# indrajeetadityaroy9/rabitq-ann-search

Hardware: AMD Instinct MI355X
Metric: qps (search_batch_device, layer-0 hot path end to end) + fastscan_dist_per_s (higher is better)
Workload: dtype u32 popcount / f32; 1 GPU; SIFT1M-class synthetic (int-valued, clustered; SURVEY 8d C2): 1000000x128 f32 (D=128), 4-bit RaBitQ FastScan + exact-L2 rerank, R=32, k=10, 10000 queries per GPU resident in HBM; n_index=1000000, dim=128, bits=4, k=10, nq_per_gpu=10000, index_builder=cphnsw_mi355x (this repo), batch_sets=2, parallelism=query-sharded x1, index replicated

## Files before the change

include/cphnsw_mi355x.h:

```cpp
#ifndef CPHNSW_MI355X_H
#define CPHNSW_MI355X_H

#include <stddef.h>
#include <stdint.h>

#ifdef __cplusplus
extern "C" {
#endif

typedef struct cph_index cph_index;

typedef enum {
    CPH_OK = 0,
    CPH_INVALID_ARGUMENT = 1,
    CPH_RUNTIME_ERROR = 2,
    CPH_OUT_OF_MEMORY = 3,
    CPH_NOT_IMPLEMENTED = 4
} cph_status;

const char* cph_last_error(void);

int cph_version(void);

int cph_create(uint64_t dim, uint64_t bits, int device, cph_index** out);
int cph_destroy(cph_index* h);

int cph_load(cph_index* h, const char* path);
int cph_save(cph_index* h, const char* path);
int cph_save_native(cph_index* h, const char* path);
int cph_load_native(cph_index* h, const char* path);
int cph_size(cph_index* h, uint64_t* n);
int cph_dim(cph_index* h, uint64_t* dim);
int cph_is_finalized(cph_index* h, int* flag);

int cph_build(cph_index* h, const float* vectors, uint64_t n);
int cph_finalize(cph_index* h);
int cph_knn_bruteforce(int device, const float* vectors, uint64_t n, uint64_t dim, const float* queries,
                       uint64_t nq, uint32_t* ids, float* dist);

int cph_encode_edges(int device, uint64_t dim, uint64_t bits, const float* parent, const float* nbrs, uint64_t cnt,
                     uint8_t* values, float* aux, uint32_t* pops);

int cph_select_hook(int device, const float* x, uint64_t n, uint64_t D, uint32_t vertex, const uint32_t* fwd,
                    const uint32_t* rev, uint64_t n_rev, uint32_t R, float alpha, float tau, float alpha_max,
                    const float* err, uint32_t* out_ids, uint32_t* out_cnt);

int cph_calib_hook(cph_index* h, const float* queries, const uint32_t* start, uint64_t ns, float* rec, uint32_t* rec_cnt,
                   float* dqp);

int cph_debug_heap_ops(int device, const uint8_t* ops, uint64_t n_ops, const float* keys, const uint32_t* ids, uint64_t n_push,
                       float* out_keys, uint32_t* out_ids, uint32_t* out_size);

int cph_search_batch(cph_index* h, const float* queries, uint64_t n, uint64_t k,
                     int64_t* ids, float* dist);

int cph_search_batch_device(cph_index* h, const float* d_queries, uint64_t n, uint64_t k,
                            int64_t* d_ids, float* d_dist, void* stream);
int cph_synchronize(cph_index* h);

typedef struct cph_filter cph_filter;
int cph_filter_create(cph_index* h, const uint32_t* words, uint64_t n_bits, cph_filter** out);
int cph_filter_destroy(cph_filter* f);
int cph_search_batch_filtered(cph_index* h, const float* queries, uint64_t n, uint64_t k, const cph_filter* f,
                              int64_t* ids, float* dist);
int cph_search_batch_device_filtered(cph_index* h, const float* d_queries, uint64_t n, uint64_t k,
                                     const cph_filter* f, int64_t* d_ids, float* d_dist, void* stream);

int cph_search_batch_exact(cph_index* h, const float* queries, uint64_t n, uint64_t k, const cph_filter* f,
                           int64_t* ids, float* dist);
int cph_search_batch_exact_device(cph_index* h, const float* d_queries, uint64_t n, uint64_t k, const cph_filter* f,
                                  int64_t* d_ids, float* d_dist, void* stream);
int cph_set_exact_threshold(cph_index* h, uint64_t max_allowed);

typedef struct cph_range cph_range;
int cph_range_search_begin(cph_index* h, const void* queries, int queries_on_device, uint64_t n, const float* radius_host,
                           const cph_filter* filter, int exact, uint64_t max_results, void* stream, cph_range** out,
                           uint64_t* total);
int cph_range_search_finish(cph_range* r, int64_t* lims_host, void* ids, void* dist, int results_on_device);
int cph_range_destroy(cph_range* r);
int cph_host_range_plan(uint64_t candidates, uint64_t n_queries, int num_cus, uint64_t* out);
int cph_host_range_tiles(const int64_t* lims, uint64_t n, uint64_t budget_bytes, uint64_t* starts_out, uint64_t* n_tiles_out);
int cph_host_range_merge_pass(const uint64_t* in, uint64_t* out, uint64_t len, uint64_t width);

int cph_search_batch_filters(cph_index* h, const float* queries, uint64_t n, uint64_t k, const cph_filter* const* filters,
                             uint32_t n_filters, const int32_t* filter_of, int exact, int64_t* ids, float* dist);
int cph_search_batch_filters_device(cph_index* h, const float* d_queries, uint64_t n, uint64_t k,
                                    const cph_filter* const* filters, uint32_t n_filters, const int32_t* filter_of, int exact,
                                    int64_t* d_ids, float* d_dist, void* stream);

int cph_filter_create_rows(cph_index* h, const uint32_t* words, uint64_t n_bits, cph_filter** out);

int cph_has_row_map(cph_index* h, int* flag);
int cph_get_row_map(cph_index* h, uint64_t first, uint64_t count, uint32_t* out);
int cph_set_row_map(cph_index* h, const uint32_t* rows, uint64_t n);
enum { CPH_IDS_INTERNAL = 0, CPH_IDS_INPUT = 1 };
int cph_set_result_ids(cph_index* h, int space);

int cph_remove(cph_index* h, const int64_t* ids, uint64_t m, int space, uint64_t* newly);
int cph_live_count(cph_index* h, uint64_t* n);
int cph_get_removed(cph_index* h, uint32_t* words);
int cph_compact(cph_index* h, int64_t* old_to_new);

int cph_search(cph_index* h, const float* query, uint64_t k, int64_t* ids, float* dist,
               uint64_t* m);

int cph_get_vectors(cph_index* h, uint64_t first, uint64_t count, float* out);

int cph_set_batch_sets(cph_index* h, uint32_t n_sets);

int cph_set_search_params(cph_index* h, uint32_t slots, uint64_t beam_capacity);

int cph_last_search_stats(cph_index* h, uint64_t out[12]);
int cph_last_query_expansions(cph_index* index, uint32_t* out, uint64_t n);
int cph_order_queries(cph_index* index, const float* keys, uint64_t n, uint32_t* order);

typedef struct cph_multi cph_multi;
int cph_multi_create(uint64_t dim, uint64_t bits, const int* devices, uint32_t n_dev, cph_multi** out);
int cph_multi_destroy(cph_multi* m);
int cph_multi_load(cph_multi* m, const char* path);
int cph_multi_load_native(cph_multi* m, const char* path);
int cph_multi_save(cph_multi* m, const char* path);
int cph_multi_save_native(cph_multi* m, const char* path);
int cph_multi_build(cph_multi* m, const float* vectors, uint64_t n);
int cph_multi_finalize(cph_multi* m);
int cph_multi_size(cph_multi* m, uint64_t* n);
int cph_multi_is_finalized(cph_multi* m, int* flag);
int cph_multi_search_batch(cph_multi* m, const float* queries, uint64_t n, uint64_t k, int64_t* ids, float* dist);
int cph_multi_search_batch_filtered(cph_multi* m, const float* queries, uint64_t n, uint64_t k,
                                    const cph_filter* const* f, int64_t* ids, float* dist);
int cph_multi_search_batch_exact(cph_multi* m, const float* queries, uint64_t n, uint64_t k,
                                 const cph_filter* const* f, int64_t* ids, float* dist);
int cph_multi_search_batch_filters(cph_multi* m, const float* queries, uint64_t n, uint64_t k, const cph_filter* const* filters,
                                   uint32_t n_filters, const int32_t* filter_of, int exact, int64_t* ids, float* dist);
typedef struct cph_multi_range cph_multi_range;
int cph_multi_range_search_begin(cph_multi* m, const float* queries, uint64_t n, const float* radius_host,
                                 const cph_filter* const* f, int exact, uint64_t max_results, cph_multi_range** out,
                                 uint64_t* total);
int cph_multi_range_search_finish(cph_multi_range* r, int64_t* lims_host, int64_t* ids, float* dist);
int cph_multi_range_destroy(cph_multi_range* r);
int cph_multi_set_exact_threshold(cph_multi* m, uint64_t max_allowed);
int cph_multi_search(cph_multi* m, const float* query, uint64_t k, int64_t* ids, float* dist, uint64_t* count);
int cph_multi_has_row_map(cph_multi* m, int* flag);
int cph_multi_set_row_map(cph_multi* m, const uint32_t* rows, uint64_t n);
int cph_multi_set_result_ids(cph_multi* m, int space);
int cph_multi_set_min_shard(cph_multi* m, uint64_t q);
int cph_multi_last_search_stats(cph_multi* m, uint64_t out[12]);
int cph_multi_last_query_expansions(cph_multi* m, uint32_t* out, uint64_t n);
int cph_multi_remove(cph_multi* m, const int64_t* ids, uint64_t cnt, int space, uint64_t* newly);
int cph_multi_live_count(cph_multi* m, uint64_t* n);
int cph_multi_get_removed(cph_multi* m, uint32_t* words);
int cph_multi_compact(cph_multi* m, int64_t* old_to_new);
int cph_multi_num_replicas(cph_multi* m, uint32_t* n);
int cph_multi_replica(cph_multi* m, uint32_t i, cph_index** out);

typedef struct cph_parts cph_parts;
typedef struct cph_parts_filter cph_parts_filter;
int cph_parts_create(uint64_t dim, uint64_t bits, const int* devices, uint32_t n_dev, cph_parts** out);
int cph_parts_destroy(cph_parts* m);
int cph_parts_build(cph_parts* m, const float* vectors, uint64_t n);
int cph_parts_finalize(cph_parts* m);
int cph_parts_size(cph_parts* m, uint64_t* n);
int cph_parts_is_finalized(cph_parts* m, int* flag);
int cph_parts_save_native(cph_parts* m, const char* path);
int cph_parts_load_native(cph_parts* m, const char* path);
int cph_parts_search_batch(cph_parts* m, const float* queries, uint64_t n, uint64_t k, int64_t* ids, float* dist);
int cph_parts_search_batch_filtered(cph_parts* m, const float* queries, uint64_t n, uint64_t k, const cph_parts_filter* f,
                                    int64_t* ids, float* dist);
int cph_parts_search_batch_exact(cph_parts* m, const float* queries, uint64_t n, uint64_t k, const cph_parts_filter* f,
                                 int64_t* ids, float* dist);
int cph_parts_search_batch_filters(cph_parts* m, const float* queries, uint64_t n, uint64_t k,
                                   const cph_parts_filter* const* filters, uint32_t n_filters, const int32_t* filter_of, int exact,
                                   int64_t* ids, float* dist);
int cph_parts_search_batch_device(cph_parts* m, const float* d_queries, uint64_t n, uint64_t k, int64_t* d_ids, float* d_dist,
                                  void* stream);
int cph_parts_search_batch_device_filtered(cph_parts* m, const float* d_queries, uint64_t n, uint64_t k, const cph_parts_filter* f,
                                           int64_t* d_ids, float* d_dist, void* stream);
int cph_parts_search_batch_exact_device(cph_parts* m, const float* d_queries, uint64_t n, uint64_t k, const cph_parts_filter* f,
                                        int64_t* d_ids, float* d_dist, void* stream);
int cph_parts_search_batch_filters_device(cph_parts* m, const float* d_queries, uint64_t n, uint64_t k,
                                          const cph_parts_filter* const* filters, uint32_t n_filters, const int32_t* filter_of,
                                          int exact, int64_t* d_ids, float* d_dist, void* stream);
int cph_parts_search(cph_parts* m, const float* query, uint64_t k, int64_t* ids, float* dist, uint64_t* count);
int cph_parts_set_exact_threshold(cph_parts* m, uint64_t max_allowed);
int cph_parts_filter_create_rows(cph_parts* m, const uint32_t* words, uint64_t n_bits, cph_parts_filter** out);
int cph_parts_filter_destroy(cph_parts_filter* f);
int cph_parts_last_search_stats(cph_parts* m, uint64_t out[13]);
int cph_parts_last_query_expansions(cph_parts* m, uint32_t* out, uint64_t n);
int cph_parts_remove(cph_parts* m, const int64_t* ids, uint64_t cnt, uint64_t* newly);
int cph_parts_live_count(cph_parts* m, uint64_t* n);
int cph_parts_get_removed(cph_parts* m, uint32_t* words);
int cph_parts_compact(cph_parts* m, int64_t* old_to_new);
int cph_parts_num_parts(cph_parts* m, uint32_t* n);
int cph_parts_part(cph_parts* m, uint32_t i, cph_index** out);
int cph_parts_bounds(cph_parts* m, uint64_t* out);
int cph_merge_rows_hook(int device, const int64_t* ids, const float* dist, uint32_t P, uint64_t n, uint64_t k, const int64_t* lo,
                        int64_t* out_ids, float* out_dist);

int cph_encode_query(cph_index* h, const float* query, uint8_t* lut, float* coeffs);

int cph_entry_point(cph_index* h, const float* query, uint32_t* entry);

int cph_fastscan_block(cph_index* h, const uint8_t* lut, const float* qparams,
                       uint32_t vertex, float dist_qp_sq, float worst, int nn_full,
                       uint32_t* sums, uint32_t* msb, float* est, float* lower,
                       float* lower_stage1);

int cph_exact_l2(cph_index* h, const float* query, const uint32_t* ids, uint64_t n,
                 float* out);

typedef struct cph_stream cph_stream;
int cph_fastscan_stream_create(int device, uint32_t D, uint32_t bits, uint64_t n_blocks,
                               uint64_t seed, cph_stream** out, uint64_t* block_bytes);
int cph_fastscan_stream_run(cph_stream* s, int reps, double* avg_ms, double* checksum);
int cph_fastscan_stream_export(cph_stream* s, uint64_t first, uint64_t count,
                               uint8_t* ref_blocks, uint8_t* lut, float* qparams,
                               float* dist_qp_sq);
int cph_fastscan_stream_eval(cph_stream* s, uint64_t first, uint64_t count, float* est,
                             float* lower);
int cph_fastscan_stream_destroy(cph_stream* s);

int cph_host_rewrite_index(const char* path_in, const char* path_out);
int cph_host_repack_block(uint32_t D, uint32_t bits, const uint8_t* ref_block, uint8_t* dev_block,
                          uint64_t* dev_bytes, uint8_t* ref_roundtrip);
int cph_host_relayout_block(uint32_t D, uint32_t bits, const uint8_t* dev_block, uint8_t* resident_block,
                            uint8_t* dev_roundtrip);
int cph_export_blocks(cph_index* h, uint64_t first, uint64_t count, int resident, uint8_t* out);
int cph_host_encode_query(uint64_t dim, const float* query, uint8_t* lut, float* coeffs, uint32_t* masks);
int cph_host_rows_filter(const uint32_t* words_in, const uint32_t* rows, uint64_t n, uint32_t* words_out);

int cph_host_live_filter(const uint32_t* words_f, const uint32_t* words_removed, uint64_t n, uint32_t* words_out,
                         uint64_t* count_out);

int cph_host_filter_ids(const uint32_t* words, uint64_t n_bits, uint32_t* out_ids, uint64_t* out_count);
int cph_host_exact_plan(uint64_t candidates, uint64_t n_queries, uint64_t k, int num_cus, uint64_t scratch_bytes, uint64_t* out);
int cph_host_filter_groups(const int32_t* filter_of, uint64_t n, const uint64_t* popcounts, uint32_t n_filters, uint64_t k,
                           int exact, uint64_t exact_threshold, uint8_t* routes, uint32_t* perm, uint32_t* seg);
int cph_host_exact_group_plan(const uint64_t* seg_candidates, const uint64_t* seg_queries, uint32_t n_segments, uint64_t k,
                              int num_cus, uint64_t scratch_bytes, uint32_t* items, uint64_t cap_items, uint64_t* out);
int cph_host_part_bounds(uint64_t n, uint32_t P, uint64_t* out);

#ifdef __cplusplus
}
#endif
#endif
```

rabitq-ann-search_amd/cphnsw_mi355x/_lib.py:

```python
import ctypes as C
import importlib.util
import os
import sys

from . import build as _build

OK, INVALID_ARGUMENT, RUNTIME_ERROR, OUT_OF_MEMORY, NOT_IMPLEMENTED = range(5)
IDS_INTERNAL, IDS_INPUT = 0, 1

SYMBOLS = {
    "cph_last_error": (C.c_char_p, []),
    "cph_version": (C.c_int, []),
    "cph_create": (C.c_int, [C.c_uint64, C.c_uint64, C.c_int, C.POINTER(C.c_void_p)]),
    "cph_destroy": (C.c_int, [C.c_void_p]),
    "cph_load": (C.c_int, [C.c_void_p, C.c_char_p]),
    "cph_save": (C.c_int, [C.c_void_p, C.c_char_p]),
    "cph_save_native": (C.c_int, [C.c_void_p, C.c_char_p]),
    "cph_load_native": (C.c_int, [C.c_void_p, C.c_char_p]),
    "cph_size": (C.c_int, [C.c_void_p, C.POINTER(C.c_uint64)]),
    "cph_dim": (C.c_int, [C.c_void_p, C.POINTER(C.c_uint64)]),
    "cph_is_finalized": (C.c_int, [C.c_void_p, C.POINTER(C.c_int)]),
    "cph_build": (C.c_int, [C.c_void_p, C.c_void_p, C.c_uint64]),
    "cph_finalize": (C.c_int, [C.c_void_p]),
    "cph_knn_bruteforce": (C.c_int, [C.c_int, C.c_void_p, C.c_uint64, C.c_uint64, C.c_void_p, C.c_uint64,
                                     C.c_void_p, C.c_void_p]),
    "cph_debug_heap_ops": (C.c_int, [C.c_int, C.c_void_p, C.c_uint64, C.c_void_p, C.c_void_p, C.c_uint64, C.c_void_p, C.c_void_p,
                                     C.c_void_p]),
    "cph_select_hook": (C.c_int, [C.c_int, C.c_void_p, C.c_uint64, C.c_uint64, C.c_uint32, C.c_void_p, C.c_void_p, C.c_uint64,
                                  C.c_uint32, C.c_float, C.c_float, C.c_float, C.c_void_p, C.c_void_p, C.c_void_p]),
    "cph_calib_hook": (C.c_int, [C.c_void_p, C.c_void_p, C.c_void_p, C.c_uint64, C.c_void_p, C.c_void_p, C.c_void_p]),
    "cph_encode_edges": (C.c_int, [C.c_int, C.c_uint64, C.c_uint64, C.c_void_p, C.c_void_p, C.c_uint64, C.c_void_p,
                                   C.c_void_p, C.c_void_p]),
    "cph_search_batch": (C.c_int, [C.c_void_p, C.c_void_p, C.c_uint64, C.c_uint64, C.c_void_p, C.c_void_p]),
    "cph_search_batch_device": (C.c_int, [C.c_void_p, C.c_void_p, C.c_uint64, C.c_uint64, C.c_void_p,
                                          C.c_void_p, C.c_void_p]),
    "cph_filter_create": (C.c_int, [C.c_void_p, C.c_void_p, C.c_uint64, C.POINTER(C.c_void_p)]),
    "cph_filter_destroy": (C.c_int, [C.c_void_p]),
    "cph_search_batch_filtered": (C.c_int, [C.c_void_p, C.c_void_p, C.c_uint64, C.c_uint64, C.c_void_p, C.c_void_p,
                                            C.c_void_p]),
    "cph_search_batch_device_filtered": (C.c_int, [C.c_void_p, C.c_void_p, C.c_uint64, C.c_uint64, C.c_void_p,
                                                   C.c_void_p, C.c_void_p, C.c_void_p]),
    "cph_search_batch_exact": (C.c_int, [C.c_void_p, C.c_void_p, C.c_uint64, C.c_uint64, C.c_void_p, C.c_void_p,
                                         C.c_void_p]),
    "cph_search_batch_exact_device": (C.c_int, [C.c_void_p, C.c_void_p, C.c_uint64, C.c_uint64, C.c_void_p,
                                                C.c_void_p, C.c_void_p, C.c_void_p]),
    "cph_set_exact_threshold": (C.c_int, [C.c_void_p, C.c_uint64]),
    "cph_search_batch_filters": (C.c_int, [C.c_void_p, C.c_void_p, C.c_uint64, C.c_uint64, C.c_void_p, C.c_uint32,
                                           C.c_void_p, C.c_int, C.c_void_p, C.c_void_p]),
    "cph_search_batch_filters_device": (C.c_int, [C.c_void_p, C.c_void_p, C.c_uint64, C.c_uint64, C.c_void_p, C.c_uint32,
                                                  C.c_void_p, C.c_int, C.c_void_p, C.c_void_p, C.c_void_p]),
    "cph_multi_search_batch_filters": (C.c_int, [C.c_void_p, C.c_void_p, C.c_uint64, C.c_uint64, C.c_void_p, C.c_uint32,
                                                 C.c_void_p, C.c_int, C.c_void_p, C.c_void_p]),
    "cph_host_filter_groups": (C.c_int, [C.c_void_p, C.c_uint64, C.c_void_p, C.c_uint32, C.c_uint64, C.c_int, C.c_uint64,
                                         C.c_void_p, C.c_void_p, C.c_void_p]),
    "cph_host_exact_group_plan": (C.c_int, [C.c_void_p, C.c_void_p, C.c_uint32, C.c_uint64, C.c_int, C.c_uint64, C.c_void_p,
                                            C.c_uint64, C.c_void_p]),
    "cph_multi_search_batch_exact": (C.c_int, [C.c_void_p, C.c_void_p, C.c_uint64, C.c_uint64, C.c_void_p,
                                               C.c_void_p, C.c_void_p]),
    "cph_multi_set_exact_threshold": (C.c_int, [C.c_void_p, C.c_uint64]),
    "cph_host_filter_ids": (C.c_int, [C.c_void_p, C.c_uint64, C.c_void_p, C.POINTER(C.c_uint64)]),
    "cph_host_exact_plan": (C.c_int, [C.c_uint64, C.c_uint64, C.c_uint64, C.c_int, C.c_uint64, C.POINTER(C.c_uint64)]),
    "cph_range_search_begin": (C.c_int, [C.c_void_p, C.c_void_p, C.c_int, C.c_uint64, C.c_void_p, C.c_void_p, C.c_int, C.c_uint64,
                                         C.c_void_p, C.POINTER(C.c_void_p), C.POINTER(C.c_uint64)]),
    "cph_range_search_finish": (C.c_int, [C.c_void_p, C.c_void_p, C.c_void_p, C.c_void_p, C.c_int]),
    "cph_range_destroy": (C.c_int, [C.c_void_p]),
    "cph_multi_range_search_begin": (C.c_int, [C.c_void_p, C.c_void_p, C.c_uint64, C.c_void_p, C.c_void_p, C.c_int, C.c_uint64,
                                               C.POINTER(C.c_void_p), C.POINTER(C.c_uint64)]),
    "cph_multi_range_search_finish": (C.c_int, [C.c_void_p, C.c_void_p, C.c_void_p, C.c_void_p]),
    "cph_multi_range_destroy": (C.c_int, [C.c_void_p]),
    "cph_host_range_plan": (C.c_int, [C.c_uint64, C.c_uint64, C.c_int, C.POINTER(C.c_uint64)]),
    "cph_host_range_tiles": (C.c_int, [C.c_void_p, C.c_uint64, C.c_uint64, C.c_void_p, C.POINTER(C.c_uint64)]),
    "cph_host_range_merge_pass": (C.c_int, [C.c_void_p, C.c_void_p, C.c_uint64, C.c_uint64]),
    "cph_filter_create_rows": (C.c_int, [C.c_void_p, C.c_void_p, C.c_uint64, C.POINTER(C.c_void_p)]),
    "cph_has_row_map": (C.c_int, [C.c_void_p, C.POINTER(C.c_int)]),
    "cph_get_row_map": (C.c_int, [C.c_void_p, C.c_uint64, C.c_uint64, C.c_void_p]),
    "cph_set_row_map": (C.c_int, [C.c_void_p, C.c_void_p, C.c_uint64]),
    "cph_set_result_ids": (C.c_int, [C.c_void_p, C.c_int]),
    "cph_remove": (C.c_int, [C.c_void_p, C.c_void_p, C.c_uint64, C.c_int, C.POINTER(C.c_uint64)]),
    "cph_live_count": (C.c_int, [C.c_void_p, C.POINTER(C.c_uint64)]),
    "cph_get_removed": (C.c_int, [C.c_void_p, C.c_void_p]),
    "cph_compact": (C.c_int, [C.c_void_p, C.c_void_p]),
    "cph_host_live_filter": (C.c_int, [C.c_void_p, C.c_void_p, C.c_uint64, C.c_void_p, C.POINTER(C.c_uint64)]),
    "cph_multi_remove": (C.c_int, [C.c_void_p, C.c_void_p, C.c_uint64, C.c_int, C.POINTER(C.c_uint64)]),
    "cph_multi_live_count": (C.c_int, [C.c_void_p, C.POINTER(C.c_uint64)]),
    "cph_multi_get_removed": (C.c_int, [C.c_void_p, C.c_void_p]),
    "cph_multi_compact": (C.c_int, [C.c_void_p, C.c_void_p]),
    "cph_parts_remove": (C.c_int, [C.c_void_p, C.c_void_p, C.c_uint64, C.POINTER(C.c_uint64)]),
    "cph_parts_live_count": (C.c_int, [C.c_void_p, C.POINTER(C.c_uint64)]),
    "cph_parts_get_removed": (C.c_int, [C.c_void_p, C.c_void_p]),
    "cph_parts_compact": (C.c_int, [C.c_void_p, C.c_void_p]),
    "cph_synchronize": (C.c_int, [C.c_void_p]),
    "cph_set_batch_sets": (C.c_int, [C.c_void_p, C.c_uint32]),
    "cph_search": (C.c_int, [C.c_void_p, C.c_void_p, C.c_uint64, C.c_void_p, C.c_void_p,
                             C.POINTER(C.c_uint64)]),
    "cph_get_vectors": (C.c_int, [C.c_void_p, C.c_uint64, C.c_uint64, C.c_void_p]),
    "cph_set_search_params": (C.c_int, [C.c_void_p, C.c_uint32, C.c_uint64]),
    "cph_last_search_stats": (C.c_int, [C.c_void_p, C.POINTER(C.c_uint64)]),
    "cph_last_query_expansions": (C.c_int, [C.c_void_p, C.c_void_p, C.c_uint64]),
    "cph_order_queries": (C.c_int, [C.c_void_p, C.c_void_p, C.c_uint64, C.c_void_p]),
    "cph_multi_create": (C.c_int, [C.c_uint64, C.c_uint64, C.c_void_p, C.c_uint32, C.POINTER(C.c_void_p)]),
    "cph_multi_destroy": (C.c_int, [C.c_void_p]),
    "cph_multi_load": (C.c_int, [C.c_void_p, C.c_char_p]),
    "cph_multi_load_native": (C.c_int, [C.c_void_p, C.c_char_p]),
    "cph_multi_save": (C.c_int, [C.c_void_p, C.c_char_p]),
    "cph_multi_save_native": (C.c_int, [C.c_void_p, C.c_char_p]),
    "cph_multi_build": (C.c_int, [C.c_void_p, C.c_void_p, C.c_uint64]),
    "cph_multi_finalize": (C.c_int, [C.c_void_p]),
    "cph_multi_size": (C.c_int, [C.c_void_p, C.POINTER(C.c_uint64)]),
    "cph_multi_is_finalized": (C.c_int, [C.c_void_p, C.POINTER(C.c_int)]),
    "cph_multi_search_batch": (C.c_int, [C.c_void_p, C.c_void_p, C.c_uint64, C.c_uint64, C.c_void_p, C.c_void_p]),
    "cph_multi_search_batch_filtered": (C.c_int, [C.c_void_p, C.c_void_p, C.c_uint64, C.c_uint64, C.c_void_p,
                                                  C.c_void_p, C.c_void_p]),
    "cph_multi_search": (C.c_int, [C.c_void_p, C.c_void_p, C.c_uint64, C.c_void_p, C.c_void_p,
                                   C.POINTER(C.c_uint64)]),
    "cph_multi_has_row_map": (C.c_int, [C.c_void_p, C.POINTER(C.c_int)]),
    "cph_multi_set_row_map": (C.c_int, [C.c_void_p, C.c_void_p, C.c_uint64]),
    "cph_multi_set_result_ids": (C.c_int, [C.c_void_p, C.c_int]),
    "cph_multi_set_min_shard": (C.c_int, [C.c_void_p, C.c_uint64]),
    "cph_multi_last_search_stats": (C.c_int, [C.c_void_p, C.POINTER(C.c_uint64)]),
    "cph_multi_last_query_expansions": (C.c_int, [C.c_void_p, C.c_void_p, C.c_uint64]),
    "cph_multi_num_replicas": (C.c_int, [C.c_void_p, C.POINTER(C.c_uint32)]),
    "cph_multi_replica": (C.c_int, [C.c_void_p, C.c_uint32, C.POINTER(C.c_void_p)]),
    "cph_parts_create": (C.c_int, [C.c_uint64, C.c_uint64, C.c_void_p, C.c_uint32, C.POINTER(C.c_void_p)]),
    "cph_parts_destroy": (C.c_int, [C.c_void_p]),
    "cph_parts_build": (C.c_int, [C.c_void_p, C.c_void_p, C.c_uint64]),
    "cph_parts_finalize": (C.c_int, [C.c_void_p]),
    "cph_parts_size": (C.c_int, [C.c_void_p, C.POINTER(C.c_uint64)]),
    "cph_parts_is_finalized": (C.c_int, [C.c_void_p, C.POINTER(C.c_int)]),
    "cph_parts_save_native": (C.c_int, [C.c_void_p, C.c_char_p]),
    "cph_parts_load_native": (C.c_int, [C.c_void_p, C.c_char_p]),
    "cph_parts_search_batch": (C.c_int, [C.c_void_p, C.c_void_p, C.c_uint64, C.c_uint64, C.c_void_p, C.c_void_p]),
    "cph_parts_search_batch_filtered": (C.c_int, [C.c_void_p, C.c_void_p, C.c_uint64, C.c_uint64, C.c_void_p, C.c_void_p,
                                                  C.c_void_p]),
    "cph_parts_search_batch_exact": (C.c_int, [C.c_void_p, C.c_void_p, C.c_uint64, C.c_uint64, C.c_void_p, C.c_void_p,
                                               C.c_void_p]),
    "cph_parts_search_batch_filters": (C.c_int, [C.c_void_p, C.c_void_p, C.c_uint64, C.c_uint64, C.c_void_p, C.c_uint32,
                                                 C.c_void_p, C.c_int, C.c_void_p, C.c_void_p]),
    "cph_parts_search_batch_device": (C.c_int, [C.c_void_p, C.c_void_p, C.c_uint64, C.c_uint64, C.c_void_p, C.c_void_p,
                                                C.c_void_p]),
    "cph_parts_search_batch_device_filtered": (C.c_int, [C.c_void_p, C.c_void_p, C.c_uint64, C.c_uint64, C.c_void_p,
                                                         C.c_void_p, C.c_void_p, C.c_void_p]),
    "cph_parts_search_batch_exact_device": (C.c_int, [C.c_void_p, C.c_void_p, C.c_uint64, C.c_uint64, C.c_void_p,
                                                      C.c_void_p, C.c_void_p, C.c_void_p]),
    "cph_parts_search_batch_filters_device": (C.c_int, [C.c_void_p, C.c_void_p, C.c_uint64, C.c_uint64, C.c_void_p, C.c_uint32,
                                                        C.c_void_p, C.c_int, C.c_void_p, C.c_void_p, C.c_void_p]),
    "cph_parts_search": (C.c_int, [C.c_void_p, C.c_void_p, C.c_uint64, C.c_void_p, C.c_void_p, C.POINTER(C.c_uint64)]),
    "cph_parts_set_exact_threshold": (C.c_int, [C.c_void_p, C.c_uint64]),
    "cph_parts_filter_create_rows": (C.c_int, [C.c_void_p, C.c_void_p, C.c_uint64, C.POINTER(C.c_void_p)]),
    "cph_parts_filter_destroy": (C.c_int, [C.c_void_p]),
    "cph_parts_last_search_stats": (C.c_int, [C.c_void_p, C.POINTER(C.c_uint64)]),
    "cph_parts_last_query_expansions": (C.c_int, [C.c_void_p, C.c_void_p, C.c_uint64]),
    "cph_parts_num_parts": (C.c_int, [C.c_void_p, C.POINTER(C.c_uint32)]),
    "cph_parts_part": (C.c_int, [C.c_void_p, C.c_uint32, C.POINTER(C.c_void_p)]),
    "cph_parts_bounds": (C.c_int, [C.c_void_p, C.c_void_p]),
    "cph_merge_rows_hook": (C.c_int, [C.c_int, C.c_void_p, C.c_void_p, C.c_uint32, C.c_uint64, C.c_uint64, C.c_void_p,
                                      C.c_void_p, C.c_void_p]),
    "cph_host_part_bounds": (C.c_int, [C.c_uint64, C.c_uint32, C.c_void_p]),
    "cph_encode_query": (C.c_int, [C.c_void_p, C.c_void_p, C.c_void_p, C.c_void_p]),
    "cph_entry_point": (C.c_int, [C.c_void_p, C.c_void_p, C.POINTER(C.c_uint32)]),
    "cph_fastscan_block": (C.c_int, [C.c_void_p, C.c_void_p, C.c_void_p, C.c_uint32, C.c_float, C.c_float,
                                     C.c_int, C.c_void_p, C.c_void_p, C.c_void_p, C.c_void_p, C.c_void_p]),
    "cph_exact_l2": (C.c_int, [C.c_void_p, C.c_void_p, C.c_void_p, C.c_uint64, C.c_void_p]),
    "cph_host_rewrite_index": (C.c_int, [C.c_char_p, C.c_char_p]),
    "cph_host_repack_block": (C.c_int, [C.c_uint32, C.c_uint32, C.c_void_p, C.c_void_p, C.POINTER(C.c_uint64), C.c_void_p]),
    "cph_host_relayout_block": (C.c_int, [C.c_uint32, C.c_uint32, C.c_void_p, C.c_void_p, C.c_void_p]),
    "cph_export_blocks": (C.c_int, [C.c_void_p, C.c_uint64, C.c_uint64, C.c_int, C.c_void_p]),
    "cph_host_encode_query": (C.c_int, [C.c_uint64, C.c_void_p, C.c_void_p, C.c_void_p, C.c_void_p]),
    "cph_host_rows_filter": (C.c_int, [C.c_void_p, C.c_void_p, C.c_uint64, C.c_void_p]),
    "cph_fastscan_stream_create": (C.c_int, [C.c_int, C.c_uint32, C.c_uint32, C.c_uint64, C.c_uint64,
                                             C.POINTER(C.c_void_p), C.POINTER(C.c_uint64)]),
    "cph_fastscan_stream_run": (C.c_int, [C.c_void_p, C.c_int, C.POINTER(C.c_double), C.POINTER(C.c_double)]),
    "cph_fastscan_stream_export": (C.c_int, [C.c_void_p, C.c_uint64, C.c_uint64, C.c_void_p, C.c_void_p,
                                             C.c_void_p, C.POINTER(C.c_float)]),
    "cph_fastscan_stream_eval": (C.c_int, [C.c_void_p, C.c_uint64, C.c_uint64, C.c_void_p, C.c_void_p]),
    "cph_fastscan_stream_destroy": (C.c_int, [C.c_void_p]),
}

_LIB = None


def _share_hip_runtime_with_torch():
    if "torch" in sys.modules:
        return
    try:
        spec = importlib.util.find_spec("torch")
    except (ImportError, ValueError):
        spec = None
    if spec is None or not spec.origin:
        return
    cand = os.path.join(os.path.dirname(spec.origin), "lib", "libamdhip64.so")
    if os.path.exists(cand):
        try:
            C.CDLL(cand, mode=C.RTLD_GLOBAL)
        except OSError:
            pass


def lib():
    global _LIB
    if _LIB is None:
        path = os.environ.get("CPH_LIB_PATH")
        if not path:
            path = _build.LIB_PATH
            if _build.needs_build():
                path = _build.build_library()
        _share_hip_runtime_with_torch()
        L = C.CDLL(path)
        diagnostic = bool(os.environ.get("CPH_LIB_PATH"))
        for name, (res, args) in SYMBOLS.items():
            try:
                fn = getattr(L, name)
            except AttributeError:
                if diagnostic:
                    continue
                raise
            fn.restype = res
            fn.argtypes = args
        _LIB = L
    return _LIB


def check(rc):
    if rc == OK:
        return
    msg = lib().cph_last_error().decode("utf-8", "replace")
    if rc == INVALID_ARGUMENT:
        raise ValueError(msg)
    if rc == OUT_OF_MEMORY:
        raise MemoryError(msg)
    if rc == NOT_IMPLEMENTED:
        raise NotImplementedError(msg)
    raise RuntimeError(msg)
```

rabitq-ann-search_amd/cphnsw_mi355x/index.py:

```python
import ctypes as C

import numpy as np

from . import _lib

DEFAULT_K = 10


def _as_f32(a):
    return np.ascontiguousarray(np.asarray(a), dtype=np.float32)


def pack_allowed_bits(mask):
    m = np.asarray(mask, dtype=bool).ravel()
    nw = (m.size + 31) // 32
    padded = np.zeros(nw * 32, dtype=np.uint64)
    padded[:m.size] = m
    return (padded.reshape(nw, 32) << np.arange(32, dtype=np.uint64)).sum(axis=1).astype(np.uint32)


class IdFilter:

    def __init__(self, index, words, n_bits, count, input_rows=False):
        self._h = C.c_void_p()
# ... 610 lines not shown
        st = np.ascontiguousarray(start, np.uint32)
        ns = q.shape[0]
        rec = np.zeros((ns, 32, 6), np.float32)
        cnt = np.zeros(ns, np.uint32)
        dqp = np.zeros(ns, np.float32)
        _lib.check(_lib.lib().cph_calib_hook(self._h, q.ctypes.data, st.ctypes.data, ns, rec.ctypes.data, cnt.ctypes.data,
                                             dqp.ctypes.data))
        return rec, cnt, dqp

    def save_native(self, path):
        if self._p is not None:
            _lib.check(_lib.lib().cph_parts_save_native(self._p, str(path).encode()))
            return
        if self._m is not None:
            _lib.check(_lib.lib().cph_multi_save_native(self._m, str(path).encode()))
            return
        _lib.check(_lib.lib().cph_save_native(self._h, str(path).encode()))

    def load_native(self, path):
        if self._p is not None:
            _lib.check(_lib.lib().cph_parts_load_native(self._p, str(path).encode()))
            return
        try:
            if self._m is not None:
                _lib.check(_lib.lib().cph_multi_load_native(self._m, str(path).encode()))
                return
            _lib.check(_lib.lib().cph_load_native(self._h, str(path).encode()))
        finally:
            self._after_index_change()

    def _after_index_change(self):
        if self._result_ids == "input" and not self.has_row_map:
            self.result_ids = "internal"

    @property
    def has_row_map(self):
        f = C.c_int(0)
        if self._p is not None:
            return self.is_finalized
        if self._m is not None:
            _lib.check(_lib.lib().cph_multi_has_row_map(self._m, C.byref(f)))
        else:
            _lib.check(_lib.lib().cph_has_row_map(self._h, C.byref(f)))
        return bool(f.value)

    def row_map(self):
        self._no_parts("row_map")
        out = np.empty(self.size, np.uint32)
        _lib.check(_lib.lib().cph_get_row_map(self._h, 0, out.size, out.ctypes.data))
        return out.astype(np.int64)

    def set_row_map(self, rows):
        self._no_parts("set_row_map")
        if rows is None:
            if self._m is not None:
                _lib.check(_lib.lib().cph_multi_set_row_map(self._m, None, 0))
            else:
                _lib.check(_lib.lib().cph_set_row_map(self._h, None, 0))
            self._result_ids = "internal"
            return
        r = np.asarray(rows)
        if r.ndim != 1 or not np.issubdtype(r.dtype, np.integer):
            raise ValueError("row map must be a 1D integer array")
        if r.size and (r.min() < 0 or r.max() > 0xFFFFFFFF):
            raise ValueError("row map must be a permutation of 0..size-1")
        r = np.ascontiguousarray(r, np.uint32)
        if self._m is not None:
            _lib.check(_lib.lib().cph_multi_set_row_map(self._m, r.ctypes.data, r.size))
        else:
            _lib.check(_lib.lib().cph_set_row_map(self._h, r.ctypes.data, r.size))

    @property
    def result_ids(self):
        return self._result_ids

    @result_ids.setter
    def result_ids(self, space):
        if space not in ("internal", "input"):
            raise ValueError('result_ids must be "internal" or "input"')
        if self._p is not None:
            if space != "input":
                raise ValueError('a partitioned index speaks input rows only: result_ids stays "input" '
                                 "(every part has its own internal ids: part(i))")
            return
        code = _lib.IDS_INPUT if space == "input" else _lib.IDS_INTERNAL
        if self._m is not None:
            _lib.check(_lib.lib().cph_multi_set_result_ids(self._m, code))
        else:
            _lib.check(_lib.lib().cph_set_result_ids(self._h, code))
        self._result_ids = space

    @property
    def exact_threshold(self):
        return self._exact_threshold

    @exact_threshold.setter
    def exact_threshold(self, max_allowed):
        v = int(max_allowed)
        if v < 0:
            raise ValueError("exact_threshold must be >= 0")
        if self._p is not None:
            _lib.check(_lib.lib().cph_parts_set_exact_threshold(self._p, v))
        elif self._m is not None:
            _lib.check(_lib.lib().cph_multi_set_exact_threshold(self._m, v))
        else:
            _lib.check(_lib.lib().cph_set_exact_threshold(self._h, v))
        self._exact_threshold = v

    @property
    def size(self):
        n = C.c_uint64(0)
        if self._p is not None:
            _lib.check(_lib.lib().cph_parts_size(self._p, C.byref(n)))
        elif self._m is not None:
            _lib.check(_lib.lib().cph_multi_size(self._m, C.byref(n)))
        else:
            _lib.check(_lib.lib().cph_size(self._h, C.byref(n)))
        return n.value

    @property
    def dim(self):
        return self._dim

    @property
    def is_finalized(self):
        f = C.c_int(0)
        if self._p is not None:
            _lib.check(_lib.lib().cph_parts_is_finalized(self._p, C.byref(f)))
        elif self._m is not None:
            _lib.check(_lib.lib().cph_multi_is_finalized(self._m, C.byref(f)))
        else:
            _lib.check(_lib.lib().cph_is_finalized(self._h, C.byref(f)))
        return bool(f.value)

    def set_batch_sets(self, n_sets):
        for h in self._replicas():
            _lib.check(_lib.lib().cph_set_batch_sets(h, int(n_sets)))

    def set_search_params(self, slots=0, beam_capacity=0):
        for h in self._replicas():
            _lib.check(_lib.lib().cph_set_search_params(h, int(slots), int(beam_capacity)))

    def last_search_stats(self):
        out = (C.c_uint64 * 13)()
        if self._p is not None:
            _lib.check(_lib.lib().cph_parts_last_search_stats(self._p, out))
        elif self._m is not None:
            _lib.check(_lib.lib().cph_multi_last_search_stats(self._m, out))
        else:
            _lib.check(_lib.lib().cph_last_search_stats(self._h, out))
        keys = ("expansions", "exact_l2", "new_neighbours", "beam_pushes", "stage2_skipped",
                "rerun_queries", "kernel_us", "expansions_nothing_new", "slots", "capacity",
                "stage2_reruns", "stage2_undecided") + (("merge_us",) if self._p is not None else ())
        return dict(zip(keys, [int(x) for x in out]))

    def synchronize(self):
        for h in self._replicas():
            _lib.check(_lib.lib().cph_synchronize(h))

    def last_query_expansions(self, n):
        out = np.empty(int(n), np.uint32)
        if self._p is not None:
            _lib.check(_lib.lib().cph_parts_last_query_expansions(self._p, out.ctypes.data, int(n)))
        elif self._m is not None:
            _lib.check(_lib.lib().cph_multi_last_query_expansions(self._m, out.ctypes.data, int(n)))
        else:
            _lib.check(_lib.lib().cph_last_query_expansions(self._h, out.ctypes.data, int(n)))
        return out

    def order_queries(self, keys):
        self._no_parts("order_queries")
        keys = np.ascontiguousarray(keys, np.float32)
        out = np.empty(len(keys), np.uint32)
        _lib.check(_lib.lib().cph_order_queries(self._h, keys.ctypes.data, len(keys), out.ctypes.data))
        return out

    def get_vectors(self, first=0, count=None):
        self._no_parts("get_vectors")
        if count is None:
            count = self.size - first
        out = np.empty((count, self._dim), np.float32)
        _lib.check(_lib.lib().cph_get_vectors(self._h, int(first), int(count), out.ctypes.data))
        return out

    def internal_to_input_rows(self, base, chunk=1 << 18):
        base = _as_f32(base)
        key = {}
        for i in range(base.shape[0] - 1, -1, -1):
            key[base[i].tobytes()] = i
        out = np.empty(self.size, np.int64)
        for lo in range(0, self.size, chunk):
            v = self.get_vectors(lo, min(chunk, self.size - lo))
            for j in range(v.shape[0]):
                out[lo + j] = key[v[j].tobytes()]
        return out

    def encode_query(self, query):
        self._no_parts("encode_query")
        q = _as_f32(query)
        D = 1
        while D < self._dim:
            D *= 2
        lut = np.zeros((D // 4, 16), np.uint8)
        co = np.zeros(3, np.float32)
        _lib.check(_lib.lib().cph_encode_query(self._h, q.ctypes.data, lut.ctypes.data, co.ctypes.data))
        return lut, co

    def entry_point(self, query):
        self._no_parts("entry_point")
        q = _as_f32(query)
        ep = C.c_uint32(0)
        _lib.check(_lib.lib().cph_entry_point(self._h, q.ctypes.data, C.byref(ep)))
        return ep.value

    def fastscan_block(self, lut, qparams, vertex, dist_qp_sq, worst=3.402823466e+38, nn_full=False):
        self._no_parts("fastscan_block")
        lut = np.ascontiguousarray(lut, np.uint8)
        qp = np.ascontiguousarray(qparams, np.float32)
        sums = np.zeros(32, np.uint32)
        msb = np.zeros(32, np.uint32)
        est = np.zeros(32, np.float32)
        lower = np.zeros(32, np.float32)
        lower1 = np.zeros(32, np.float32)
        _lib.check(_lib.lib().cph_fastscan_block(
            self._h, lut.ctypes.data, qp.ctypes.data, int(vertex), float(dist_qp_sq), float(worst),
            int(bool(nn_full)), sums.ctypes.data, msb.ctypes.data, est.ctypes.data, lower.ctypes.data,
            lower1.ctypes.data))
        return sums, msb, est, lower, lower1

    def exact_l2(self, query, ids):
        self._no_parts("exact_l2")
        q = _as_f32(query)
        ids = np.ascontiguousarray(ids, np.uint32)
        out = np.zeros(len(ids), np.float32)
        _lib.check(_lib.lib().cph_exact_l2(self._h, q.ctypes.data, ids.ctypes.data, len(ids),
                                           out.ctypes.data))
        return out


def knn_bruteforce(vectors, queries=None, device=None):
    v = _as_f32(vectors)
    n, dim = v.shape
    q = None if queries is None else _as_f32(queries)
    if q is not None and (q.ndim != 2 or q.shape[1] != dim):
        raise ValueError("queries must be a (nq, dim) array")
    rows = n if q is None else q.shape[0]
    ids = np.zeros((rows, 32), np.uint32)
    dist = np.zeros((rows, 32), np.float32)
    dev = _default_device() if device is None else int(device)
    _lib.check(_lib.lib().cph_knn_bruteforce(dev, v.ctypes.data, n, dim, None if q is None else q.ctypes.data,
                                             0 if q is None else q.shape[0], ids.ctypes.data, dist.ctypes.data))
    return ids, dist


def encode_edges(parent, nbrs, bits, device=None):
    p = _as_f32(parent)
    nb = _as_f32(nbrs)
    cnt, dim = nb.shape
    D = 16
    while D < dim:
        D *= 2
    vals = np.zeros((cnt, D), np.uint8)
    aux = np.zeros((cnt, 3), np.float32)
    pops = np.zeros((cnt, 2), np.uint32)
    dev = _default_device() if device is None else int(device)
    _lib.check(_lib.lib().cph_encode_edges(dev, dim, int(bits), p.ctypes.data, nb.ctypes.data, cnt, vals.ctypes.data,
                                           aux.ctypes.data, pops.ctypes.data))
    return vals, aux, pops


def select_neighbors_debug(x, vertex, fwd, rev, R, alpha, tau, alpha_max=0.0, err=None, device=None):
    x = _as_f32(x)
    n, D = x.shape
    fwd = np.ascontiguousarray(fwd, np.uint32)
    rev = np.ascontiguousarray(rev, np.uint32)
    assert fwd.shape == (32,)
    out = np.zeros(32, np.uint32)
    cnt = np.zeros(1, np.uint32)
    e = None if err is None else _as_f32(err)
    dev = _default_device() if device is None else int(device)
    _lib.check(_lib.lib().cph_select_hook(dev, x.ctypes.data, n, D, int(vertex), fwd.ctypes.data, rev.ctypes.data if len(rev) else None,
                                          len(rev), int(R), float(alpha), float(tau), float(alpha_max),
                                          None if e is None else e.ctypes.data, out.ctypes.data, cnt.ctypes.data))
    return out[:cnt[0]].copy()


def heap_ops_debug(ops, keys, ids, device=None):
    ops = np.ascontiguousarray(ops, np.uint8)
    keys = np.ascontiguousarray(keys, np.float32)
    ids = np.ascontiguousarray(ids, np.uint32)
    n_push = int((ops != 0).sum())
    assert len(keys) == n_push and len(ids) == n_push
    ok = np.zeros(max(1, n_push), np.float32)
    oi = np.zeros(max(1, n_push), np.uint32)
    sz = np.zeros(1, np.uint32)
    dev = _default_device() if device is None else int(device)
    _lib.check(_lib.lib().cph_debug_heap_ops(dev, ops.ctypes.data, len(ops), keys.ctypes.data, ids.ctypes.data, n_push,
                                             ok.ctypes.data, oi.ctypes.data, sz.ctypes.data))
    return ok[:sz[0]].copy(), oi[:sz[0]].copy()


def _default_device():
    import os
    try:
        return int(os.environ.get("LOCAL_RANK", "0"))
    except ValueError:
        return 0
# ... 46 lines not shown
```

rabitq-ann-search_amd/csrc/cphnsw_mi355x.hip:

```cpp
#include <hip/hip_runtime.h>

#include <algorithm>
#include <atomic>
#include <cfloat>
#include <chrono>
#include <condition_variable>
#include <deque>
#include <functional>
#include <memory>
#include <mutex>
#include <new>
#include <shared_mutex>
#include <string>
#include <thread>
#include <vector>

#include "../../include/cphnsw_mi355x.h"
#include "cph_core.h"
#include "device_buf.h"
#include "device_encode.h"
#include "device_fastscan.h"
#include "device_search.h"
#include "device_stream.h"
#include "device_heap_test.h"
#include "device_relayout.h"
#include "device_rows.h"
#include "device_tombstone.h"
#include "device_exact.h"
#include "device_range.h"
#include "host_index.h"
#include "host_parallel.h"
#include "search_coalescer.h"
#include "multi_device.h"
#include "partitioned.h"
#include "device_merge.h"
#include "native_file.h"
#include "builder_pipeline.h"

using namespace cph;

namespace {

thread_local std::string g_err;

int fail(int code, const std::string& msg) {
    g_err = msg;
    return code;
}

struct InvalidArg : std::invalid_argument {
    using std::invalid_argument::invalid_argument;
};

template <class F>
int guarded(F&& f) {
    try {
        f();
        return CPH_OK;
    } catch (const std::invalid_argument& e) {
        return fail(CPH_INVALID_ARGUMENT, e.what());
    } catch (const std::bad_alloc&) {
        return fail(CPH_OUT_OF_MEMORY, "out of memory");
    } catch (const std::exception& e) {
        return fail(CPH_RUNTIME_ERROR, e.what());
    }
}

size_t next_pow2(size_t n) {
    size_t p = 1;
    while (p < n) p *= 2;
    return p;
}

#define CPH_LAUNCH_BITS(KERNEL, bits, SDV, grid, block, lds, st, args)                            \
    do {                                                                                          \
        if ((bits) == 1) hipLaunchKernelGGL((KERNEL<1, SDV>), grid, block, lds, st, args);        \
        else if ((bits) == 2) hipLaunchKernelGGL((KERNEL<2, SDV>), grid, block, lds, st, args);   \
        else hipLaunchKernelGGL((KERNEL<4, SDV>), grid, block, lds, st, args);                    \
    } while (0)
#define CPH_LAUNCH(KERNEL, bits, D, grid, block, lds, st, args)                                   \
    do {                                                                                          \
        if ((D) == 128) CPH_LAUNCH_BITS(KERNEL, bits, 128, grid, block, lds, st, args);           \
        else if ((D) == 1024) CPH_LAUNCH_BITS(KERNEL, bits, 1024, grid, block, lds, st, args);    \
        else CPH_LAUNCH_BITS(KERNEL, bits, 0, grid, block, lds, st, args);                        \
        HIP_CHECK(hipGetLastError());                                                             \
    } while (0)

__global__ void scan_counts_kernel(const uint8_t* blocks, uint64_t n, uint32_t stride, uint32_t count_off, uint32_t* flags) {
    const uint64_t v = (uint64_t)blockIdx.x * blockDim.x + threadIdx.x;
    if (v >= n) return;
    const uint32_t cnt = *reinterpret_cast<const uint32_t*>(blocks + v * stride + count_off);
    if (cnt & 7u) atomicOr(flags, 2u);
}

}

struct BatchSet {
    DevBuf<float> d_queries_raw, d_queries, d_entry_dist, d_dist;
    DevBuf<uint4> d_qmasks;
    DevBuf<QueryHeader> d_qhdr;
    DevBuf<int64_t> d_ids;
    DevBuf<uint32_t> d_count, d_status, d_order, d_redo;
    DevBuf<unsigned long long> d_stats;
    unsigned long long* pin_stats = nullptr;
    uint8_t* pin_io = nullptr;
    uint8_t* pin_io_dev = nullptr;
    size_t pin_io_bytes = 0;
    DevBuf<uint32_t> d_bitmaps, d_logids;
    DevBuf<uint32_t> d_beam, d_beam_tail;
    uint32_t slots = 0;
    uint64_t cap = 0;
    DevBuf<uint32_t> r_bitmaps, r_logids;
    DevBuf<uint32_t> r_beam, r_beam_tail;
    uint32_t r_slots = 0;
    hipEvent_t ev0 = nullptr, ev1 = nullptr, ev_done = nullptr;
    bool used = false;
    uint32_t nq = 0;
    uint32_t run_slots = 0;
    uint64_t run_cap = 0;
    DevBuf<float> x_qpad, x_qnorm;
    DevBuf<unsigned long long> x_pools;
    DevBuf<uint32_t> x_counts;
    bool stats_in_hbm = false;
    uint8_t* pin_tab = nullptr;
    size_t pin_tab_bytes = 0;
    DevBuf<uint8_t> d_tab;
    DevBuf<uint32_t> d_redo2;
    hipEvent_t ev_tab = nullptr;
    bool tab_used = false;
};
constexpr int kMaxBatchSets = 4;

struct RangeScratch {
    DevBuf<float> d_q, qpad, qnorm, d_rad, g_dist, o_dist;
    DevBuf<int64_t> g_ids, o_ids;
    DevBuf<uint32_t> counts;
    DevBuf<unsigned long long> offs, sums, d_lims, d_stats, arena, arena2;
    DevBuf<uint8_t> d_tab;
};
constexpr size_t kRangeScratchKept = 2;
constexpr uint64_t kSmallBatch = 32;

struct cph_filter {
    int device = 0;
    uint64_t n_bits = 0;
    uint64_t popcount = 0;
    DevBuf<uint32_t> words;
    mutable std::mutex ids_mu;
    mutable DevBuf<uint32_t> ids, ids_scratch;
    mutable hipEvent_t ids_ev = nullptr;
    mutable std::mutex eff_mu;
    mutable std::vector<std::pair<uint64_t, std::shared_ptr<cph_filter>>> eff;
    ~cph_filter() { if (ids_ev) (void)hipEventDestroy(ids_ev); }
};
constexpr size_t kEffCached = 4;
struct EffDeleter {
    void operator()(cph_filter* f) const {
        if (hipSetDevice(f->device) == hipSuccess) (void)hipDeviceSynchronize();
        delete f;
    }
};
static std::atomic<uint64_t> g_removed_epoch{0};

struct cph_index {
    uint64_t dim = 0;
    uint32_t bits = 0;
    uint32_t D = 0;
    int device = 0;
    bool finalized = false;
    bool needs_build = false;
    bool borrowed = false;
    bool host_less = false;
    std::vector<float> pending;
    uint64_t pending_n = 0;
    HostIndex host;
    DevLayout L{};
    SearchConsts sc{};
    uint32_t flags = 0;
    int num_cus = 256;
    bool waves_from_env = false;
    uint32_t waves_per_cu = 4 * CPH_SEARCH_WAVES_PER_SIMD;
    DevBuf<uint8_t> d_blocks;
    DevBuf<float> d_raw, d_norm;
    DevBuf<uint32_t> d_rows;
    bool has_rows = false;
    bool ids_input = false;
    size_t exact_scratch_bytes = (size_t)1 << 30;
    uint64_t exact_threshold = 0;
    DevBuf<uint32_t> d_removed;
    DevBuf<unsigned long long> d_rm_count;
    uint64_t rm_epoch = 0;
    std::shared_ptr<cph_filter> live;
    std::atomic<bool> tombstones{false};
    DevBuf<float> d_signs;
    DevBuf<uint32_t> d_upper;
    DevBuf<uint32_t> d_row_of;
    UpperLayerDev layers[kMaxUpperLayers];
    int32_t dev_max_level = 0;
    float norm_factor = 0.0f, inv_sqrt_d = 0.0f;
    NativeMapping native_map;
    const uint8_t* own_view = nullptr;
    std::vector<uint8_t> own_store;
    BatchSet sets[kMaxBatchSets + kLeaderSlots];
    int n_sets = 2;
    int last_set = kMaxBatchSets - 1;
    int last_search = -1;
    bool last_range = false;
    uint64_t range_exact = 0;
    std::vector<std::unique_ptr<RangeScratch>> range_scratch;
    uint64_t index_epoch = 0;
    hipStream_t own_stream = nullptr;
    bool order_queries = true;
    uint32_t want_slots = 0;
    uint64_t want_cap = 0;
    uint64_t auto_cap = 0;
    bool pf_off = false;
    bool pf_dense = false;
    std::mutex mu;
    SearchCoalescer coal;
    struct LeaderSlot {
        hipStream_t stream = nullptr;
        uint8_t* pin = nullptr;
        uint8_t* pin_dev = nullptr;
        size_t pin_bytes = 0;
        uint32_t seq = 0;
        uint64_t cur_n = 0, cur_k = 0;
    } leaders[kLeaderSlots];

    void use_device() const { HIP_CHECK(hipSetDevice(device)); }
};

namespace {

bool probe_first(const cph_index* h) {
    return (h->L.D == 128 || h->L.D == 1024) && !(h->flags & 2u) && !h->pf_off && !h->pf_dense;
}

uint64_t stage2_stat(const BatchSet& s, StatWord w) {
#if defined(CPH_PHASE_TIMERS) || defined(CPH_TRAFFIC_STATS)
    (void)s; (void)w;
    return 0;
#else
    return s.pin_stats[w];
#endif
}

void reset_adaptation(cph_index* h) {
    h->auto_cap = 0;
    h->pf_off = false;
    h->pf_dense = false;
    h->last_search = -1;
    h->last_range = false;
}

void drop_host_state(cph_index* h) {
    h->needs_build = false;
    std::vector<float>().swap(h->pending);
    h->pending_n = 0;
    h->native_map.reset();
    h->own_view = nullptr;
    std::vector<uint8_t>().swap(h->own_store);
}

void sync_row_map(cph_index* h) {
    const std::vector<uint32_t>& rows = h->host.rows;
    h->has_rows = !rows.empty();
    if (h->has_rows) {
        h->d_rows.alloc(rows.size());
        HIP_CHECK(hipMemcpy(h->d_rows.p, rows.data(), rows.size() * 4, hipMemcpyHostToDevice));
    } else {
        h->d_rows.release();
        h->ids_input = false;
    }
}

hipStream_t own_stream(cph_index* h);

std::shared_ptr<cph_filter> make_live_filter(cph_index* h, const uint32_t* d_allow) {
    const uint64_t n = h->host.n, nw = (n + 31) / 32;
    std::shared_ptr<cph_filter> e(new cph_filter(), EffDeleter());
    e->device = h->device;
    e->n_bits = n;
    e->words.alloc(std::max<uint64_t>(nw, 1));
    h->d_rm_count.alloc(1);
    hipStream_t st = own_stream(h);
    live_filter(d_allow, h->d_removed.p, n, e->words.p, h->d_rm_count.p, st);
    unsigned long long c = 0;
    HIP_CHECK(hipMemcpyAsync(&c, h->d_rm_count.p, 8, hipMemcpyDeviceToHost, st));
    HIP_CHECK(hipStreamSynchronize(st));
    e->popcount = c;
    return e;
}

void sync_removed(cph_index* h) {
    HostIndex& hi = h->host;
    h->rm_epoch = ++g_removed_epoch;
    h->live.reset();
    if (hi.n_removed == 0) {
        std::vector<uint32_t>().swap(hi.removed);
        h->d_removed.release();
        h->tombstones.store(false);
        return;
    }
    h->tombstones.store(true);
    const uint64_t nw = (hi.n + 31) / 32;
    h->d_removed.alloc(nw);
    HIP_CHECK(hipMemcpy(h->d_removed.p, hi.removed.data(), nw * 4, hipMemcpyHostToDevice));
    h->live = make_live_filter(h, nullptr);
}

std::shared_ptr<const cph_filter> effective_filter(cph_index* h, const cph_filter* f) {
    if (h->host.n_removed == 0) return std::shared_ptr<const cph_filter>(std::shared_ptr<const cph_filter>(), f);
    if (!f) {
        if (!h->live) h->live = make_live_filter(h, nullptr);
        return h->live;
    }
    std::lock_guard<std::mutex> lk(f->eff_mu);
    for (auto& e : f->eff)
        if (e.first == h->rm_epoch) return e.second;
    if (f->eff.size() >= kEffCached) f->eff.erase(f->eff.begin());
    std::shared_ptr<cph_filter> e = make_live_filter(h, f->words.p);
    f->eff.emplace_back(h->rm_epoch, e);
    return e;
}

void require_finalized(cph_index* h) {
    if (!h->finalized) throw std::runtime_error("Search failed: invalid entry point after finalize.");
}

void release_scratch(BatchSet& s) {
    s.d_bitmaps.release(); s.d_logids.release(); s.d_beam.release(); s.d_beam_tail.release();
    s.r_bitmaps.release(); s.r_logids.release(); s.r_beam.release(); s.r_beam_tail.release();
    s.x_qpad.release(); s.x_qnorm.release(); s.x_pools.release(); s.x_counts.release();
    s.slots = 0; s.cap = 0; s.r_slots = 0;
}

void quiesce(cph_index* h) {
    for (auto& s : h->sets)
        if (s.used && s.ev_done) HIP_CHECK(hipEventSynchronize(s.ev_done));
}

void upload_arrays(cph_index* h) {
    h->use_device();
    quiesce(h);
    const HostIndex& hi = h->host;
    h->L = make_dev_layout((uint32_t)hi.D, (uint32_t)hi.bw);
    const size_t n = hi.n;
    const size_t stride = h->L.stride;
    h->d_blocks.alloc(n * stride + 64);
    h->d_raw.alloc(n * hi.D);
    h->d_norm.alloc(n);
    const size_t chunk = std::max<size_t>(1, std::min<size_t>(n, (256u << 20) / stride));
    std::vector<uint8_t> stage(chunk * stride);
    for (size_t base = 0; base < n; base += chunk) {
        const size_t cnt = std::min(chunk, n - base);
        parallel_for(cnt, 256, [&](size_t lo, size_t hi_) {
            for (size_t v = lo; v < hi_; ++v)
                repack_ref_to_dev(hi.nb(base + v), hi.RL, h->L, &stage[v * stride]);
        });
        HIP_CHECK(hipMemcpy(h->d_blocks.p + base * stride, stage.data(), cnt * stride,
                            hipMemcpyHostToDevice));
    }
    relayout_blocks(h->d_blocks.p, n, h->L, true);
    HIP_CHECK(hipMemcpy(h->d_raw.p, hi.raw.data(), n * hi.D * 4, hipMemcpyHostToDevice));
    HIP_CHECK(hipMemcpy(h->d_norm.p, hi.norm_sq.data(), n * 4, hipMemcpyHostToDevice));
}

void upload_feeders(cph_index* h) {
    h->use_device();
    quiesce(h);
    const HostIndex& hi = h->host;
    const size_t n = hi.n;
    h->L = make_dev_layout((uint32_t)hi.D, (uint32_t)hi.bw);
    h->sc = hi.consts();
    h->flags = hi.has_dup_neighbors ? 1u : 0u;
    if (n != 0) {
        DevBuf<uint32_t> d_flag(1);
        HIP_CHECK(hipMemset(d_flag.p, 0, 4));
        hipLaunchKernelGGL(scan_counts_kernel, dim3((uint32_t)((n + 255) / 256)), dim3(256), 0, nullptr, h->d_blocks.p, (uint64_t)n,
                           h->L.stride, h->L.count_off, d_flag.p);
        HIP_CHECK(hipGetLastError());
        uint32_t f = 0;
        HIP_CHECK(hipMemcpy(&f, d_flag.p, 4, hipMemcpyDeviceToHost));
        h->flags |= f & 2u;
    }
    h->d_signs.alloc(3 * hi.D);
    HIP_CHECK(hipMemcpy(h->d_signs.p, hi.rot.signs.data(), 3 * hi.D * 4, hipMemcpyHostToDevice));
    const float d = static_cast<float>(hi.D);
    h->norm_factor = 1.0f / (d * std::sqrt(d));
    h->inv_sqrt_d = 1.0f / std::sqrt(d);
    const int nl = std::min<int>({(int)hi.upper.size(), (int)hi.max_level, kMaxUpperLayers});
    h->dev_max_level = hi.max_level > 0 ? nl : 0;
    std::vector<uint32_t> flat;
    std::vector<size_t> off_nodes(nl), off_offs(nl), off_nbrs(nl);
    for (int l = 0; l < nl; ++l) {
        const auto& layer = hi.upper[l];
        off_nodes[l] = flat.size();
        for (const auto& e : layer) flat.push_back(e.node);
        off_offs[l] = flat.size();
        uint32_t acc = 0;
        for (const auto& e : layer) { flat.push_back(acc); acc += (uint32_t)e.nbrs.size(); }
        flat.push_back(acc);
        off_nbrs[l] = flat.size();
        for (const auto& e : layer) flat.insert(flat.end(), e.nbrs.begin(), e.nbrs.end());
    }
    h->d_upper.alloc(flat.size() + 1);
    if (!flat.empty())
        HIP_CHECK(hipMemcpy(h->d_upper.p, flat.data(), flat.size() * 4, hipMemcpyHostToDevice));
    for (int l = 0; l < kMaxUpperLayers; ++l) h->layers[l] = UpperLayerDev{nullptr, nullptr, nullptr, nullptr, 0};
    int mapped = 0;
    for (int l = 0; l < nl; ++l) mapped += hi.upper[l].size() > 16 ? 1 : 0;
    h->d_row_of.alloc((size_t)mapped * n + 1);
    std::vector<uint32_t> row_of;
    for (int l = 0, m = 0; l < nl; ++l) {
        const uint32_t* dmap = nullptr;
        if (hi.upper[l].size() > 16) {
            row_of.assign(n, kInvalidNode);
            uint64_t first = 0;
            bool fits = true;
            for (size_t r = 0; r < hi.upper[l].size(); ++r) {
                const uint64_t deg = hi.upper[l][r].nbrs.size();
                if (first >= (1u << 26) || deg > 62) { fits = false; break; }
                row_of[hi.upper[l][r].node] = (uint32_t)first | ((uint32_t)deg << 26);
                first += deg;
            }
            if (!fits) { h->layers[l] = UpperLayerDev{h->d_upper.p + off_nodes[l], h->d_upper.p + off_offs[l], h->d_upper.p + off_nbrs[l], nullptr, (uint32_t)hi.upper[l].size()}; ++m; continue; }
            HIP_CHECK(hipMemcpy(h->d_row_of.p + (size_t)m * n, row_of.data(), n * 4, hipMemcpyHostToDevice));
            dmap = h->d_row_of.p + (size_t)m * n;
            ++m;
        }
        h->layers[l] = UpperLayerDev{h->d_upper.p + off_nodes[l], h->d_upper.p + off_offs[l],
                                     h->d_upper.p + off_nbrs[l], dmap, (uint32_t)hi.upper[l].size()};
    }
    for (auto& s : h->sets) release_scratch(s);
    reset_adaptation(h);
}

void materialize_search_data(cph_index* h) {
    HostIndex& hi = h->host;
    if (!hi.search_data.empty() || hi.n == 0) return;
    h->use_device();
    quiesce(h);
    const size_t n = hi.n, stride = h->L.stride, own_stride = hi.RL.nb_off;
    hi.search_data.assign(n * hi.RL.vertex_bytes, 0);
    const size_t chunk = std::max<size_t>(1, std::min<size_t>(n, (512u << 20) / stride));
    std::vector<uint8_t> stage(chunk * stride);
    for (size_t base = 0; base < n; base += chunk) {
        const size_t c = std::min(chunk, n - base);
        download_blocks(h->d_blocks.p + base * stride, c, h->L, stage.data());
        parallel_for(c, 256, [&](size_t lo, size_t hi_) {
            for (size_t v = lo; v < hi_; ++v) {
                uint8_t* dst = &hi.search_data[(base + v) * hi.RL.vertex_bytes];
                if (h->own_view) std::memcpy(dst, h->own_view + (base + v) * own_stride, own_stride);
                repack_dev_to_ref(&stage[v * stride], h->L, hi.RL, dst + hi.RL.nb_off);
            }
        });
    }
}

void init_set(BatchSet& s) {
    if (s.ev0) return;
    HIP_CHECK(hipEventCreate(&s.ev0));
    HIP_CHECK(hipEventCreate(&s.ev1));
    HIP_CHECK(hipEventCreateWithFlags(&s.ev_done, hipEventDisableTiming));
    HIP_CHECK(hipHostMalloc(reinterpret_cast<void**>(&s.pin_stats), kStatWords * 8, hipHostMallocDefault));
    std::memset(s.pin_stats, 0, kStatWords * 8);
}

BatchSet& next_set(cph_index* h, hipStream_t st) {
    h->last_set = (h->last_set + 1) % h->n_sets;
    BatchSet& s = h->sets[h->last_set];
    init_set(s);
    for (BatchSet& o : h->sets) {
        if (!(o.used && o.ev_done && !o.stats_in_hbm && hipEventQuery(o.ev_done) == hipSuccess)) continue;
        const uint64_t reruns = o.pin_stats[kStatReruns], stage2_reruns = stage2_stat(o, kStatStage2Reruns);
        if (reruns > stage2_reruns && o.cap < h->host.n + 1)
            h->auto_cap = std::max<uint64_t>(h->auto_cap, std::min<uint64_t>(h->host.n + 1, o.cap * 4));
        if (stage2_reruns * 50 > o.nq) h->pf_off = true;
        if (o.pin_stats[kStatExpansions] >= 10000) {
            const double new_per_exp = (double)o.pin_stats[kStatNew] / (double)o.pin_stats[kStatExpansions];
            const double off = h->bits == 4 ? 6.0 : 2.8, on = h->bits == 4 ? 4.5 : 2.2;
            if (new_per_exp > off) h->pf_dense = true;
            else if (new_per_exp < on) h->pf_dense = false;
        }
    }
    if (s.used) HIP_CHECK(hipStreamWaitEvent(st, s.ev_done, 0));
    return s;
}

void stage_queries(cph_index* h, BatchSet& s, const float* d_raw_q, uint64_t nq, hipStream_t st) {
    const HostIndex& hi = h->host;
    const uint32_t D = (uint32_t)hi.D, PW = h->L.PW;
    if (hi.entry == kInvalidNode || hi.entry >= hi.n)
        throw std::runtime_error("Search failed: invalid entry point after finalize.");
    if (s.d_queries.n < nq * D || s.d_qmasks.n < nq * PW || s.d_qhdr.n < nq) {
        if (s.used) HIP_CHECK(hipEventSynchronize(s.ev_done));
        s.d_queries.alloc(nq * D);
        s.d_qmasks.alloc(nq * PW);
        s.d_qhdr.alloc(nq);
        s.d_entry_dist.alloc(nq);
        s.d_order.alloc(nq);
    }
    EncodeArgs a{};
    a.queries_raw = d_raw_q;
    a.nq = (uint32_t)nq;
    a.dim = (uint32_t)hi.dim;
    a.D = D;
    a.PW = PW;
    a.signs = h->d_signs.p;
    a.norm_factor = h->norm_factor;
    a.inv_sqrt_d = h->inv_sqrt_d;
    a.raw = h->d_raw.p;
    a.n = hi.n;
    a.entry = hi.entry;
    a.max_level = h->dev_max_level;
    for (int l = 0; l < kMaxUpperLayers; ++l) a.layers[l] = h->layers[l];
    a.queries_padded = s.d_queries.p;
    a.qmasks = s.d_qmasks.p;
    a.qhdr = s.d_qhdr.p;
    a.entry_dist = s.d_entry_dist.p;
    const uint32_t grid = (uint32_t)std::min<uint64_t>(nq, (uint64_t)h->num_cus * 32);
    hipLaunchKernelGGL(encode_kernel, dim3(grid), dim3(64), encode_lds_bytes(D), st, a);
    HIP_CHECK(hipGetLastError());
}

const float* upload_queries(cph_index* h, BatchSet& s, const float* queries, uint64_t nq, hipStream_t st) {
    if (s.d_queries_raw.n < nq * h->dim) {
        if (s.used) HIP_CHECK(hipEventSynchronize(s.ev_done));
        s.d_queries_raw.alloc(nq * h->dim);
    }
    HIP_CHECK(hipMemcpyAsync(s.d_queries_raw.p, queries, nq * h->dim * 4, hipMemcpyHostToDevice, st));
    return s.d_queries_raw.p;
}

void ensure_scratch(cph_index* h, BatchSet& s, uint32_t slots, uint64_t cap, hipStream_t st) {
    const uint64_t n = h->host.n;
    const uint64_t bm_words = (n + 31) / 32;
    if (!(s.slots >= slots && s.cap == cap)) {
        if (s.used) HIP_CHECK(hipEventSynchronize(s.ev_done));
        s.d_bitmaps.alloc((size_t)slots * bm_words);
        HIP_CHECK(hipMemsetAsync(s.d_bitmaps.p, 0, (size_t)slots * bm_words * 4, st));
        s.d_logids.alloc((size_t)slots * cap);
        s.d_beam.alloc((size_t)slots * kBeamPagesDwords);
        s.d_beam_tail.alloc((size_t)slots * beam_tail_dwords(cap));
        s.slots = slots;
        s.cap = cap;
    }
    if ((cap < n + 1 || probe_first(h)) && s.r_slots == 0) {
        size_t free_b = 0, total_b = 0;
        HIP_CHECK(hipMemGetInfo(&free_b, &total_b));
        const uint64_t per = (n + 1) * 4 + ((uint64_t)kBeamPagesDwords + beam_tail_dwords(n + 1)) * 4 + bm_words * 4;
        const uint64_t want = (&s - h->sets) >= kMaxBatchSets ? kLeaderGroup : kSmallBatch;
        const uint32_t rs = (uint32_t)std::max<uint64_t>(1, std::min<uint64_t>(want, (uint64_t)(free_b * 0.25) / per));
        s.r_bitmaps.alloc((size_t)rs * bm_words);
        HIP_CHECK(hipMemsetAsync(s.r_bitmaps.p, 0, (size_t)rs * bm_words * 4, st));
        s.r_logids.alloc((size_t)rs * (n + 1));
        s.r_beam.alloc((size_t)rs * kBeamPagesDwords);
        s.r_beam_tail.alloc((size_t)rs * beam_tail_dwords(n + 1));
        s.r_slots = rs;
    }
}

struct DoneFlags {
    uint32_t* flags = nullptr;
    uint32_t seq = 0;
};

enum class Launch {
    Main,
    Rerun,
    Direct,
};

void launch_search_kernel(uint32_t bits, uint32_t D, bool pf, bool filtered, bool table_of_filters, uint32_t grid, size_t lds,
                          hipStream_t st, const SearchArgs& a) {
    using Kernel = void (*)(SearchArgs);
    static const Kernel table[3][3][4] = {
        {{search_kernel<1, 0, true, false>, search_kernel<1, 0, true, false>, search_kernel<1, 0, false, true>,
          search_kernel<1, 0, false, true, true>},
         {search_kernel<1, 128, false, false>, search_kernel<1, 128, true, false>, search_kernel<1, 128, false, true>,
          search_kernel<1, 128, false, true, true>},
         {search_kernel<1, 1024, false, false>, search_kernel<1, 1024, true, false>, search_kernel<1, 1024, false, true>,
          search_kernel<1, 1024, false, true, true>}},
        {{search_kernel<2, 0, true, false>, search_kernel<2, 0, true, false>, search_kernel<2, 0, false, true>,
          search_kernel<2, 0, false, true, true>},
         {search_kernel<2, 128, false, false>, search_kernel<2, 128, true, false>, search_kernel<2, 128, false, true>,
          search_kernel<2, 128, false, true, true>},
         {search_kernel<2, 1024, false, false>, search_kernel<2, 1024, true, false>, search_kernel<2, 1024, false, true>,
          search_kernel<2, 1024, false, true, true>}},
        {{search_kernel<4, 0, true, false>, search_kernel<4, 0, true, false>, search_kernel<4, 0, false, true>,
          search_kernel<4, 0, false, true, true>},
         {search_kernel<4, 128, false, false>, search_kernel<4, 128, true, false>, search_kernel<4, 128, false, true>,
          search_kernel<4, 128, false, true, true>},
         {search_kernel<4, 1024, false, false>, search_kernel<4, 1024, true, false>, search_kernel<4, 1024, false, true>,
          search_kernel<4, 1024, false, true, true>}},
    };
    const Kernel kernel = table[bits == 1 ? 0 : bits == 2 ? 1 : 2][D == 128 ? 1 : D == 1024 ? 2 : 0][table_of_filters ? 3 : filtered ? 2 : pf ? 1 : 0];
    hipLaunchKernelGGL(kernel, dim3(grid), dim3(64), lds, st, a);
    HIP_CHECK(hipGetLastError());
}

struct SubBatch {
    const uint32_t* todo = nullptr;
    int queue = 0;
    uint32_t* redo = nullptr;
    const uint32_t* const* allow_tab = nullptr;
    const uint32_t* filter_of = nullptr;
};

void launch_search(cph_index* h, BatchSet& s, uint32_t nq, uint32_t k, int64_t* d_ids, float* d_dist, uint32_t* d_count,
                   const uint32_t* d_todo, Launch mode, hipStream_t st, DoneFlags done = DoneFlags(),
                   const uint32_t* d_allow = nullptr, const SubBatch* sub = nullptr) {
    const uint64_t n = h->host.n;
    const bool tab = sub && sub->allow_tab;
    const bool pf = mode == Launch::Main && d_allow == nullptr && !tab && probe_first(h);
    SearchArgs a{};
    a.allow = d_allow;
    if (tab) { a.allow_tab = sub->allow_tab; a.filter_of = sub->filter_of; }
    a.rows = h->ids_input ? h->d_rows.p : nullptr;
    a.done_flags = done.flags;
    a.done_seq = done.seq;
    a.blocks = h->d_blocks.p;
    a.raw = h->d_raw.p;
    a.norm_sq = h->d_norm.p;
    a.n = n;
    a.L = h->L;
    a.flags = h->flags;
    a.queries = s.d_queries.p;
    a.qmasks = s.d_qmasks.p;
    a.qhdr = s.d_qhdr.p;
    a.k = k;
    a.sc = h->sc;
    a.bm_words = (n + 31) / 32;
    a.out_ids = d_ids;
    a.out_dist = d_dist;
    a.out_count = d_count;
    a.status = s.d_status.p;
    a.stats = s.d_stats.p;
    if (mode == Launch::Main) {
        a.cap = s.cap;
        a.bitmaps = s.d_bitmaps.p;
        a.beam_pages = s.d_beam.p;
        a.beam_tail = s.d_beam_tail.p;
        a.log_ids = s.d_logids.p;
    } else {
        a.cap = n + 1;
        a.bitmaps = s.r_bitmaps.p;
        a.beam_pages = s.r_beam.p;
        a.beam_tail = s.r_beam_tail.p;
        a.log_ids = s.r_logids.p;
    }
    uint32_t* queue = reinterpret_cast<uint32_t*>(s.d_stats.p + kStatQueues) + (sub ? sub->queue : 0);
    uint32_t* const d_redo = sub ? sub->redo : s.d_redo.p;
    uint32_t grid = 0;
    switch (mode) {
    case Launch::Main:
        a.todo = d_todo;
        a.nq = nq;
        a.counter = queue + kQueueMain;
        a.redo = (s.cap < n + 1 || pf) ? d_redo : nullptr;
        a.redo_count = queue + kQueueRerunLen;
        grid = std::min(s.run_slots, nq);
        break;
    case Launch::Rerun:
        a.todo = d_redo;
        a.nq_dev = queue + kQueueRerunLen;
        a.counter = queue + kQueueRerun;
        grid = s.r_slots;
        break;
    case Launch::Direct:
        a.todo = d_todo;
        a.nq = nq;
        a.counter = queue + kQueueMain;
        grid = nq;
        break;
    }
    const size_t lds = search_lds_bytes(h->L.D, h->L.PW, k);
    if (lds > 160 * 1024) throw InvalidArg("k too large for the on-chip result heap");
    launch_search_kernel(h->bits, h->L.D, pf, d_allow != nullptr, tab, grid, lds, st, a);
}

void finish_batch(cph_index* h, BatchSet& s, hipStream_t st) {
    HIP_CHECK(hipEventRecord(s.ev1, st));
    s.stats_in_hbm = (&s - h->sets) >= kMaxBatchSets;
    if (!s.stats_in_hbm) HIP_CHECK(hipMemcpyAsync(s.pin_stats, s.d_stats.p, kStatWords * 8, hipMemcpyDeviceToHost, st));
    HIP_CHECK(hipEventRecord(s.ev_done, st));
    s.used = true;
    h->last_search = (int)(&s - h->sets);
    h->last_range = false;
}

bool size_search(cph_index* h, BatchSet& s, uint32_t nq, uint32_t k, hipStream_t st) {
    const uint64_t n = h->host.n;
    uint32_t wpc = h->waves_per_cu;
    if (!h->waves_from_env) {
        wpc = 4 * (uint32_t)search_waves_per_simd(search_static_d(h->L.D) ? (int)h->L.D : 0, (int)h->bits);
        const size_t lds_wave = search_lds_bytes(h->L.D, h->L.PW, k);
        wpc = (uint32_t)std::max<size_t>(1, std::min<size_t>(wpc, (160u * 1024u) / lds_wave));
    }
    uint32_t max_slots = h->want_slots ? h->want_slots : (uint32_t)h->num_cus * wpc;
    if (!h->want_slots && h->n_sets > 2) max_slots = std::max<uint32_t>(64, max_slots / 2);
    const uint32_t rounds = (nq + max_slots - 1) / max_slots;
    uint32_t slots = std::min<uint32_t>(nq, (nq + rounds - 1) / rounds);
    const bool ordered = h->dev_max_level > 0 && h->order_queries;
    if (ordered) {
        slots = std::min<uint32_t>(nq, max_slots);
        if (!h->want_slots && nq > max_slots / 2) slots = std::min<uint32_t>(max_slots, nq - nq / 8);
    }
    const uint64_t bm_bytes = ((n + 31) / 32) * 4;
    uint64_t cap = h->want_cap ? h->want_cap : std::max<uint64_t>(h->auto_cap, std::min<uint64_t>(n + 1, 1u << 16));
    cap = std::max<uint64_t>(64, std::min<uint64_t>(cap, n + 1));
    if (!(s.slots >= slots && s.cap == cap)) {
        size_t free_b = 0, total_b = 0;
        HIP_CHECK(hipMemGetInfo(&free_b, &total_b));
        auto slot_bytes = [&](uint64_t c) { return c * 4 + ((uint64_t)kBeamPagesDwords + beam_tail_dwords(c)) * 4 + bm_bytes; };
        const uint64_t held = (uint64_t)s.slots * slot_bytes(s.cap);
        const uint64_t budget = (uint64_t)((free_b + held) * 0.3);
        while (slots > 64 && (uint64_t)slots * slot_bytes(cap) > budget) slots /= 2;
        while (cap > 4096 && (uint64_t)slots * slot_bytes(cap) > budget) cap /= 2;
    }
    ensure_scratch(h, s, slots, cap, st);
    slots = std::min(slots, s.slots);
    s.run_slots = slots;
    s.run_cap = s.cap;
    return ordered;
}

void enqueue_search(cph_index* h, BatchSet& s, uint32_t nq, uint32_t k, int64_t* d_ids, float* d_dist,
                    hipStream_t st, uint32_t* d_count_out = nullptr, DoneFlags done = DoneFlags(),
                    const cph_filter* filter = nullptr) {
    const uint64_t n = h->host.n;
    if (s.d_count.n < nq) {
        if (s.used) HIP_CHECK(hipEventSynchronize(s.ev_done));
        s.d_count.alloc(nq);
        s.d_status.alloc(nq);
        s.d_redo.alloc(nq);
    }
    s.d_stats.alloc(kStatWords);
    HIP_CHECK(hipMemsetAsync(s.d_stats.p, 0, kStatWords * 8, st));
    if (filter && filter->popcount == 0) {
        uint32_t* d_count = d_count_out ? d_count_out : s.d_count.p;
        HIP_CHECK(hipEventRecord(s.ev0, st));
        HIP_CHECK(hipMemsetAsync(d_ids, 0xFF, (size_t)nq * k * 8, st));
        HIP_CHECK(hipMemsetD32Async(reinterpret_cast<hipDeviceptr_t>(d_dist), (int)0x7F7FFFFF, (size_t)nq * k, st));
        HIP_CHECK(hipMemsetAsync(d_count, 0, (size_t)nq * 4, st));
        HIP_CHECK(hipMemsetAsync(s.d_status.p, 0, (size_t)nq * 4, st));
        s.run_slots = 0;
        s.run_cap = 0;
        s.nq = nq;
        finish_batch(h, s, st);
        return;
    }
    const uint32_t* d_allow = filter ? filter->words.p : nullptr;
    const bool ordered = size_search(h, s, nq, k, st);
    const uint32_t slots = s.run_slots;
    s.nq = nq;
    const uint32_t* d_order = nullptr;
    if (nq > slots && ordered) {
        hipLaunchKernelGGL(order_kernel, dim3(1), dim3(1024), 0, st, s.d_entry_dist.p, nq, s.d_order.p);
        HIP_CHECK(hipGetLastError());
        d_order = s.d_order.p;
    }
    uint32_t* d_count = d_count_out ? d_count_out : s.d_count.p;
    HIP_CHECK(hipEventRecord(s.ev0, st));
    const bool rerun = s.cap < n + 1 || (d_allow == nullptr && probe_first(h));
    if (rerun && nq <= s.r_slots && !h->want_cap && !h->want_slots) {
        s.run_slots = nq;
        s.run_cap = n + 1;
        launch_search(h, s, nq, k, d_ids, d_dist, d_count, nullptr, Launch::Direct, st, done, d_allow);
    } else {
        launch_search(h, s, nq, k, d_ids, d_dist, d_count, d_order, Launch::Main, st, done, d_allow);
        if (rerun) launch_search(h, s, nq, k, d_ids, d_dist, d_count, nullptr, Launch::Rerun, st, done, d_allow);
    }
    finish_batch(h, s, st);
}

hipStream_t own_stream(cph_index* h) {
    if (!h->own_stream) HIP_CHECK(hipStreamCreateWithFlags(&h->own_stream, hipStreamNonBlocking));
    return h->own_stream;
}

constexpr size_t kFlagBytes = kLeaderGroup * 4;
struct PinnedIo {
    size_t o_ids, o_dist, o_cnt, o_q, need;
    PinnedIo(uint64_t n, uint64_t k, uint64_t dim, size_t prefix) {
        o_ids = prefix;
        o_dist = o_ids + n * k * 8;
        o_cnt = o_dist + n * k * 4;
        o_q = (o_cnt + n * 4 + 15) & ~(size_t)15;
        need = o_q + n * dim * 4;
    }
    int64_t* ids(uint8_t* base) const { return reinterpret_cast<int64_t*>(base + o_ids); }
    float* dist(uint8_t* base) const { return reinterpret_cast<float*>(base + o_dist); }
    uint32_t* counts(uint8_t* base) const { return reinterpret_cast<uint32_t*>(base + o_cnt); }
    float* queries(uint8_t* base) const { return reinterpret_cast<float*>(base + o_q); }
};

bool grow_pinned(uint8_t*& host, uint8_t*& dev, size_t& bytes, size_t need) {
    if (bytes >= need) return false;
    if (host) HIP_CHECK(hipHostFree(host));
    host = nullptr;
    bytes = 0;
    const size_t want = std::max<size_t>(need * 2, 64 * 1024);
    HIP_CHECK(hipHostMalloc(reinterpret_cast<void**>(&host), want, hipHostMallocMapped | hipHostMallocCoherent));
    HIP_CHECK(hipHostGetDevicePointer(reinterpret_cast<void**>(&dev), host, 0));
    bytes = want;
    return true;
}

void check_filter(const cph_index* h, const cph_filter* f) {
    if (f->device != h->device) throw InvalidArg("filter belongs to another device");
    if (f->n_bits != h->host.n)
        throw InvalidArg("filter covers " + std::to_string(f->n_bits) + " ids, the index holds " + std::to_string(h->host.n));
}

bool batch_has_work(cph_index* h, const cph_filter* f, const float* queries, uint64_t n, uint64_t k, const int64_t* ids,
                    const float* dist) {
    require_finalized(h);
    if (f) check_filter(h, f);
    if (n == 0 || k == 0) return false;
    if (n > 0xFFFFFFFFull || k > 0xFFFFFFFFull) throw InvalidArg("batch too large");
    if (!queries || !ids || !dist) throw InvalidArg("null argument");
    return true;
}

const uint32_t* filter_id_list(const cph_filter* f, hipStream_t st) {
    std::lock_guard<std::mutex> lk(f->ids_mu);
    if (!f->ids_ev) {
        f->ids.alloc(f->popcount);
        f->ids_scratch.alloc((f->n_bits + kFilterSpan - 1) / kFilterSpan);
        filter_ids(f->words.p, f->n_bits, f->ids_scratch.p, f->ids.p, st);
        hipEvent_t ev = nullptr;
        HIP_CHECK(hipEventCreateWithFlags(&ev, hipEventDisableTiming));
        HIP_CHECK(hipEventRecord(ev, st));
        f->ids_ev = ev;
    } else {
        HIP_CHECK(hipStreamWaitEvent(st, f->ids_ev, 0));
    }
    return f->ids.p;
}

void enqueue_exact(cph_index* h, BatchSet& s, const float* d_raw_q, uint32_t nq, uint32_t k, const cph_filter* filter,
                   int64_t* d_ids, float* d_dist, hipStream_t st) {
    const uint64_t n = h->host.n, m = filter ? filter->popcount : n;
    const uint32_t D = h->L.D;
    const uint32_t nq_pad = (nq + kExactQT - 1) / kExactQT * kExactQT;
    const ExactPlan pl = plan_exact(m, nq, k, h->num_cus, h->exact_scratch_bytes);
    if (s.x_qpad.n < (size_t)nq_pad * D || s.x_pools.n < pl.pool_keys || s.x_counts.n < (size_t)pl.P * pl.tile_q || s.d_status.n < nq) {
        if (s.used) HIP_CHECK(hipEventSynchronize(s.ev_done));
        s.x_qpad.alloc((size_t)nq_pad * D);
        s.x_qnorm.alloc(nq_pad);
        s.x_pools.alloc(pl.pool_keys);
        s.x_counts.alloc((size_t)pl.P * pl.tile_q);
        s.d_count.alloc(nq);
        s.d_status.alloc(nq);
        s.d_redo.alloc(nq);
    }
    const uint32_t* d_list = filter ? filter_id_list(filter, st) : nullptr;
    s.d_stats.alloc(kStatWords);
    HIP_CHECK(hipMemsetAsync(s.d_stats.p, 0, kStatWords * 8, st));
    HIP_CHECK(hipMemsetAsync(s.d_status.p, 0, (size_t)nq * 4, st));
    HIP_CHECK(hipEventRecord(s.ev0, st));
    hipLaunchKernelGGL(exact_pad_kernel, dim3(std::min<uint32_t>(nq_pad, (uint32_t)h->num_cus * 16)), dim3(64), 0, st, d_raw_q, nq,
                       nq_pad, (uint32_t)h->dim, D, s.x_qpad.p, s.x_qnorm.p, s.d_stats.p, (unsigned long long)nq * m);
    HIP_CHECK(hipGetLastError());
    ExactArgs a{};
    a.raw = h->d_raw.p;
    a.norm_sq = h->d_norm.p;
    a.ids = d_list;
    a.m = (uint32_t)m;
    a.D = D;
    a.qpad = s.x_qpad.p;
    a.qnorm = s.x_qnorm.p;
    a.gq = pl.gq;
    a.part = pl.part;
    a.k = k;
    a.C = pl.C;
    a.pools = s.x_pools.p;
    a.counts = s.x_counts.p;
    for (uint32_t q0 = 0; q0 < nq; q0 += pl.tile_q) {
        a.q_first = q0;
        a.q_count = std::min(pl.tile_q, nq - q0);
        const dim3 grid(pl.P, (a.q_count + pl.gq - 1) / pl.gq);
        launch_exact_scan(D, grid, (size_t)pl.C * 8 + (size_t)pl.gq * 8, st, a);
        hipLaunchKernelGGL(exact_merge_kernel, dim3(a.q_count), dim3(64), (size_t)pl.C * 8, st, (const unsigned long long*)s.x_pools.p,
                           (const uint32_t*)s.x_counts.p, pl.P, a.q_first, a.q_count, k, pl.C,
                           (const uint32_t*)(h->ids_input ? h->d_rows.p : nullptr), d_ids, d_dist);
        HIP_CHECK(hipGetLastError());
    }
    s.run_slots = 0;
    s.run_cap = 0;
    s.nq = nq;
// ... 250 lines not shown
                           s.d_stats.p, n_exact);
        HIP_CHECK(hipGetLastError());
        ExactGroupArgs a{};
        a.raw = h->d_raw.p;
        a.norm_sq = h->d_norm.p;
        a.D = D;
        a.qpad = s.x_qpad.p;
        a.qnorm = s.x_qnorm.p;
        a.gq = pl.gq;
        a.k = k;
        a.C = pl.C;
        a.pools = s.x_pools.p;
        a.counts = s.x_counts.p;
        for (size_t l = 0; l < n_launch; ++l) {
            a.items = reinterpret_cast<const ExactItem*>(dt + o_items) + pl.launch_items[l];
            launch_exact_scan_groups(D, pl.launch_items[l + 1] - pl.launch_items[l], (size_t)pl.C * 8 + (size_t)pl.gq * 8, st, a);
            hipLaunchKernelGGL(exact_merge_groups_kernel, dim3(l_qhi[l] - l_qlo[l]), dim3(64), (size_t)pl.C * 8, st,
                               (const unsigned long long*)s.x_pools.p, (const uint32_t*)s.x_counts.p,
                               reinterpret_cast<const uint4*>(dt + o_desc) + l_qlo[l], k, pl.C, d_rows, d_ids, d_dist);
            HIP_CHECK(hipGetLastError());
        }
    }
    if (n_pad) {
        hipLaunchKernelGGL(exact_fill_rows_kernel, dim3(n_pad), dim3(64), 0, st, reinterpret_cast<const uint32_t*>(dt + o_pad), k, d_ids, d_dist);
        HIP_CHECK(hipGetLastError());
    }
    s.run_slots = 0;
    s.run_cap = 0;
    if (n_gf + n_gp) {
        stage_queries(h, s, d_raw_q, nq, st);
        const bool ordered = size_search(h, s, std::max(n_gf, n_gp), k, st);
        const uint32_t* d_order = nullptr;
        if (std::max(n_gf, n_gp) == nq && nq > s.run_slots && ordered) {
            hipLaunchKernelGGL(order_kernel, dim3(1), dim3(1024), 0, st, s.d_entry_dist.p, nq, s.d_order.p);
            HIP_CHECK(hipGetLastError());
            d_order = s.d_order.p;
        }
        bool any_main = false;
        uint32_t direct_slots = 0;
        auto run = [&](uint32_t cnt, const uint32_t* list, SubBatch sub) {
            if (!cnt) return;
            sub.todo = cnt == nq ? d_order : list;
            const bool rerun = s.cap < n + 1 || (!sub.allow_tab && probe_first(h));
            if (rerun && cnt <= s.r_slots && !h->want_cap && !h->want_slots) {
                direct_slots = std::max(direct_slots, cnt);
                launch_search(h, s, cnt, k, d_ids, d_dist, s.d_count.p, sub.todo, Launch::Direct, st, DoneFlags(), nullptr, &sub);
            } else {
                any_main = true;
                launch_search(h, s, cnt, k, d_ids, d_dist, s.d_count.p, sub.todo, Launch::Main, st, DoneFlags(), nullptr, &sub);
                if (rerun) launch_search(h, s, cnt, k, d_ids, d_dist, s.d_count.p, nullptr, Launch::Rerun, st, DoneFlags(), nullptr, &sub);
            }
        };
        SubBatch filtered, plain;
        filtered.queue = 0;
        filtered.redo = s.d_redo.p;
        filtered.allow_tab = reinterpret_cast<const uint32_t* const*>(dt + o_tab);
        filtered.filter_of = reinterpret_cast<const uint32_t*>(dt + o_fof);
        plain.queue = kQueueSecond;
        plain.redo = s.d_redo2.p;
        run(n_gf, reinterpret_cast<const uint32_t*>(dt + o_gf), filtered);
        run(n_gp, reinterpret_cast<const uint32_t*>(dt + o_gp), plain);
        if (!any_main) {
            s.run_slots = direct_slots;
            s.run_cap = n + 1;
        }
    }
    s.nq = nq;
    finish_batch(h, s, st);
}

void search_batch_filters_host(cph_index* h, const float* queries, uint64_t n, uint64_t k, const cph_filter* const* filters, uint32_t F,
                               const int32_t* filter_of, bool exact, int64_t* ids, float* dist) {
    if (!h) throw InvalidArg("null handle");
    std::lock_guard<std::mutex> lk(h->mu);
    if (!filters_batch_has_work(h, filters, F, filter_of, queries, n, k, ids, dist)) return;
    LiveFilters lf;
    live_filters(h, filters, F, filter_of, n, lf);
    filters = lf.filters; F = lf.F; filter_of = lf.filter_of;
    const FilterGroups g = group_filters(h, filters, F, filter_of, n, k, exact);
    h->use_device();
    hipStream_t st = own_stream(h);
    BatchSet& s = next_set(h, st);
    const float* d_q = upload_queries(h, s, queries, n, st);
    if (s.d_ids.n < n * k) {
        if (s.used) HIP_CHECK(hipEventSynchronize(s.ev_done));
        s.d_ids.alloc(n * k);
        s.d_dist.alloc(n * k);
    }
    enqueue_filters(h, s, d_q, (uint32_t)n, (uint32_t)k, filters, F, filter_of, g, s.d_ids.p, s.d_dist.p, st);
    HIP_CHECK(hipMemcpyAsync(ids, s.d_ids.p, n * k * 8, hipMemcpyDeviceToHost, st));
    HIP_CHECK(hipMemcpyAsync(dist, s.d_dist.p, n * k * 4, hipMemcpyDeviceToHost, st));
    HIP_CHECK(hipEventRecord(s.ev_done, st));
    HIP_CHECK(hipStreamSynchronize(st));
}

void search_batch_filters_device(cph_index* h, const float* d_queries, uint64_t n, uint64_t k, const cph_filter* const* filters,
                                 uint32_t F, const int32_t* filter_of, bool exact, int64_t* d_ids, float* d_dist, void* stream) {
    if (!h) throw InvalidArg("null handle");
    std::lock_guard<std::mutex> lk(h->mu);
    if (!filters_batch_has_work(h, filters, F, filter_of, d_queries, n, k, d_ids, d_dist)) return;
    LiveFilters lf;
    live_filters(h, filters, F, filter_of, n, lf);
    filters = lf.filters; F = lf.F; filter_of = lf.filter_of;
    const FilterGroups g = group_filters(h, filters, F, filter_of, n, k, exact);
    h->use_device();
    hipStream_t st = reinterpret_cast<hipStream_t>(stream);
    BatchSet& s = next_set(h, st);
    enqueue_filters(h, s, d_queries, (uint32_t)n, (uint32_t)k, filters, F, filter_of, g, d_ids, d_dist, st);
}

}

#ifdef CPH_SEARCH_TRACE
static std::atomic<uint64_t> g_tr[6];
static inline uint64_t now_ns() { return std::chrono::duration_cast<std::chrono::nanoseconds>(std::chrono::steady_clock::now().time_since_epoch()).count(); }
#define CPH_TR(i, v) g_tr[i] += (v)
#else
#define CPH_TR(i, v) ((void)(v))
static inline uint64_t now_ns() { return 0; }
#endif

extern "C" {

const char* cph_last_error(void) { return g_err.c_str(); }
int cph_version(void) { return 104; }

int cph_create(uint64_t dim, uint64_t bits, int device, cph_index** out) {
    return guarded([&] {
        if (!out) throw InvalidArg("out must not be null");
        *out = nullptr;
        if (bits != 1 && bits != 2 && bits != 4)
            throw InvalidArg("Unsupported bits=" + std::to_string(bits) + ". Supported: 1, 2, 4.");
        const size_t pd = next_pow2(dim);
        if (dim == 0) throw InvalidArg("dim must be > 0");
        if (pd < 16 || pd > 2048)
            throw InvalidArg("Unsupported dimension " + std::to_string(dim) + " (padded to " + std::to_string(pd) +
                             "). Supported padded dims: 16, 32, 64, 128, 256, 512, 1024, 2048.");
        int ndev = 0;
        if (hipGetDeviceCount(&ndev) != hipSuccess || ndev <= 0)
            throw std::runtime_error("No HIP device available: the MI355X path has no CPU fallback.");
        if (device < 0 || device >= ndev) throw InvalidArg("invalid device ordinal");
        auto* h = new cph_index();
        h->dim = dim;
        h->bits = (uint32_t)bits;
        h->D = (uint32_t)pd;
        h->device = device;
        hipDeviceProp_t prop;
        if (hipGetDeviceProperties(&prop, device) == hipSuccess) h->num_cus = prop.multiProcessorCount;
        if (const char* e = getenv("CPH_QUERY_ORDER")) h->order_queries = atoi(e) != 0;
        if (const char* e = getenv("CPH_LEADER_SLOTS")) h->coal.n_slots = std::max(1, std::min(kLeaderSlots, atoi(e)));
        if (const char* e = getenv("CPH_EXACT_SCRATCH_MB")) h->exact_scratch_bytes = (size_t)std::max(1, atoi(e)) << 20;
        if (const char* e = getenv("CPH_GATHER_US")) h->coal.gather_us = std::max(0, atoi(e));
        if (const char* e = getenv("CPH_WAVES_PER_CU")) { h->waves_per_cu = (uint32_t)std::max(1, atoi(e)); h->waves_from_env = true; }
        *out = h;
    });
}

}

static void refuse_borrowed(const cph_index* h, const char* what) {
    if (h->borrowed)
        throw InvalidArg(std::string(what) + " on a replica of a multi-device index: call it on the multi-device handle");
}
static void refuse_host_less(const cph_index* h, const char* what) {
    if (h->host_less)
        throw InvalidArg(std::string(what) + " on a replica that keeps no host arrays: use replica 0");
}

static void destroy_index(cph_index* h) {
    (void)hipSetDevice(h->device);
    for (auto& s : h->sets) {
        if (s.used && s.ev_done) (void)hipEventSynchronize(s.ev_done);
        if (s.ev0) (void)hipEventDestroy(s.ev0);
        if (s.ev1) (void)hipEventDestroy(s.ev1);
        if (s.ev_done) (void)hipEventDestroy(s.ev_done);
        if (s.pin_stats) (void)hipHostFree(s.pin_stats);
        if (s.pin_io) (void)hipHostFree(s.pin_io);
        if (s.pin_tab) (void)hipHostFree(s.pin_tab);
        if (s.ev_tab) (void)hipEventDestroy(s.ev_tab);
    }
#ifdef CPH_SEARCH_TRACE
    if (g_tr[0]) fprintf(stderr, "[search trace] groups=%llu callers=%llu per group: mutex wait %.1f us, enqueue %.1f us; per caller: own-query wait %.1f us\n",
                         (unsigned long long)g_tr[0], (unsigned long long)g_tr[1], g_tr[2] / 1e3 / g_tr[0], g_tr[3] / 1e3 / g_tr[0], g_tr[4] / 1e3 / g_tr[1]);
    for (auto& x : g_tr) x = 0;
#endif
    if (h->own_stream) (void)hipStreamDestroy(h->own_stream);
    for (auto& ls : h->leaders) {
        if (ls.stream) { (void)hipStreamSynchronize(ls.stream); (void)hipStreamDestroy(ls.stream); }
        if (ls.pin) (void)hipHostFree(ls.pin);
    }
    delete h;
}

extern "C" int cph_destroy(cph_index* h) {
    return guarded([&] {
        if (!h) return;
        refuse_borrowed(h, "cph_destroy");
        destroy_index(h);
    });
}

static void begin_device_swap(cph_index* h) {
    h->use_device();
    quiesce(h);
    h->finalized = false;
    for (auto& s : h->sets) release_scratch(s);
    h->last_search = -1;
    h->last_range = false;
    h->range_scratch.clear();
    ++h->index_epoch;
}

static void load_v2(cph_index* h, const char* path) {
    std::lock_guard<std::mutex> lk(h->mu);
    HostIndex t;
    t.load(path, h->D, h->bits, h->dim);
    begin_device_swap(h);
    h->host = std::move(t);
    drop_host_state(h);
    upload_arrays(h);
    sync_row_map(h);
    sync_removed(h);
    upload_feeders(h);
    h->finalized = true;
}

extern "C" {

int cph_load(cph_index* h, const char* path) {
    return guarded([&] {
        if (!h || !path) throw InvalidArg("null argument");
        refuse_borrowed(h, "cph_load");
        load_v2(h, path);
    });
}

int cph_save(cph_index* h, const char* path) {
    return guarded([&] {
        if (!h || !path) throw InvalidArg("null argument");
        refuse_host_less(h, "cph_save");
        std::lock_guard<std::mutex> lk(h->mu);
        if (!h->finalized) throw std::runtime_error("Index must be finalized before saving.");
        if (h->host.n_removed != 0)
            throw std::runtime_error("The reference format cannot carry removed rows (" + std::to_string(h->host.n_removed) +
                                     " here) and a file without them would bring them back: compact() the index first, or use save_native.");
        materialize_search_data(h);
        h->host.save(path);
    });
}

int cph_save_native(cph_index* h, const char* path) {
    return guarded([&] {
        if (!h || !path) throw InvalidArg("null argument");
        refuse_host_less(h, "cph_save_native");
        std::lock_guard<std::mutex> lk(h->mu);
        if (!h->finalized) throw std::runtime_error("Index must be finalized before saving.");
        h->use_device();
        quiesce(h);
        const HostIndex& hi = h->host;
        const size_t n = hi.n, stride = h->L.stride, own_stride = hi.RL.nb_off;
        std::vector<uint8_t> blocks(n * stride), own;
        download_blocks(h->d_blocks.p, n, h->L, blocks.data());
        const uint8_t* own_p = h->own_view;
        if (!own_p) {
            own.resize(n * own_stride);
            for (size_t v = 0; v < n; ++v) std::memcpy(&own[v * own_stride], &hi.search_data[v * hi.RL.vertex_bytes], own_stride);
            own_p = own.data();
        }
        write_native(path, hi, (uint32_t)stride, own_p, (uint32_t)own_stride, blocks.data());
    });
}

}

struct NativeLoaded {
    HostIndex t;
    NativeMapping map;
    NativeHeader nh;
};

static void read_native_for(const cph_index* h, const char* path, NativeLoaded& out) {
    out.nh = read_native(path, h->D, h->bits, h->dim, out.t, out.map);
}

static void install_native(cph_index* h, NativeLoaded& in) {
    std::lock_guard<std::mutex> lk(h->mu);
    HostIndex& t = in.t;
    NativeMapping& map = in.map;
    const NativeHeader nh = in.nh;
    begin_device_swap(h);
    h->host = std::move(t);
    drop_host_state(h);
    h->native_map = std::move(map);
    const uint8_t* base = static_cast<const uint8_t*>(h->native_map.base);
    h->own_view = base + nh.own_off;
    h->L = make_dev_layout((uint32_t)h->host.D, (uint32_t)h->host.bw);
    const size_t n = h->host.n;
    h->d_blocks.alloc(n * nh.stride + 64);
    h->d_raw.alloc(n * h->host.D);
    h->d_norm.alloc(n);
    HIP_CHECK(hipMemcpy(h->d_blocks.p, base + nh.blocks_off, n * (size_t)nh.stride, hipMemcpyHostToDevice));
    relayout_blocks(h->d_blocks.p, n, h->L, true);
    HIP_CHECK(hipMemcpy(h->d_raw.p, h->host.raw_view, n * h->host.D * 4, hipMemcpyHostToDevice));
    HIP_CHECK(hipMemcpy(h->d_norm.p, h->host.norm_sq.data(), n * 4, hipMemcpyHostToDevice));
    sync_row_map(h);
    sync_removed(h);
// ... 202 lines not shown
        a.L = L; a.blocks = d_blocks.p;
        a.dbg_values = d_vals.p; a.dbg_aux = d_aux.p; a.dbg_pops = d_pops.p;
        build::run_encode(bits, a, 1, 1);
        HIP_CHECK(hipMemcpy(values, d_vals.p, cnt * D, hipMemcpyDeviceToHost));
        HIP_CHECK(hipMemcpy(aux, d_aux.p, cnt * 3 * 4, hipMemcpyDeviceToHost));
        HIP_CHECK(hipMemcpy(pops, d_pops.p, cnt * 2 * 4, hipMemcpyDeviceToHost));
    });
}

int cph_select_hook(int device, const float* x, uint64_t n, uint64_t D, uint32_t vertex, const uint32_t* fwd,
                    const uint32_t* rev, uint64_t n_rev, uint32_t R, float alpha, float tau, float alpha_max,
                    const float* err, uint32_t* out_ids, uint32_t* out_cnt) {
    return guarded([&] {
        if (!x || !fwd || !out_ids || !out_cnt || n == 0 || vertex >= n) throw InvalidArg("bad arguments");
        if (D < 16 || D > 2048 || (D & (D - 1))) throw InvalidArg("D must be a power of two in 16..2048");
        if (R == 0 || R > 32 || n_rev > 96) throw InvalidArg("R must be 1..32 and n_rev <= 96 (the hub path is not a unit case)");
        for (int i = 0; i < 32; ++i)
            if (fwd[i] != kInvalidNode && fwd[i] >= n) throw InvalidArg("candidate out of range");
        for (uint64_t i = 0; i < n_rev; ++i)
            if (rev[i] >= n) throw InvalidArg("candidate out of range");
        HIP_CHECK(hipSetDevice(device));
        DevBuf<float> d_x(n * D), d_err(n);
        DevBuf<uint32_t> d_fwd(32), d_rev(std::max<uint64_t>(1, n_rev)), d_rows(std::max<uint64_t>(1, n_rev) + 1), d_out(32), d_cnt(1);
        DevBuf<uint64_t> d_off(2);
        HIP_CHECK(hipMemcpy(d_x.p, x, n * D * 4, hipMemcpyHostToDevice));
        if (err) HIP_CHECK(hipMemcpy(d_err.p, err, n * 4, hipMemcpyHostToDevice));
        HIP_CHECK(hipMemcpy(d_fwd.p, fwd, 128, hipMemcpyHostToDevice));
        std::vector<uint32_t> rows(n_rev + 1), revrows(std::max<uint64_t>(1, n_rev));
        rows[0] = vertex;
        for (uint64_t i = 0; i < n_rev; ++i) { rows[i + 1] = rev[i]; revrows[i] = (uint32_t)(i + 1); }
        HIP_CHECK(hipMemcpy(d_rows.p, rows.data(), rows.size() * 4, hipMemcpyHostToDevice));
        HIP_CHECK(hipMemcpy(d_rev.p, revrows.data(), revrows.size() * 4, hipMemcpyHostToDevice));
        const uint64_t off[2] = {0, n_rev};
        HIP_CHECK(hipMemcpy(d_off.p, off, 16, hipMemcpyHostToDevice));
        build::SelectArgs a{};
        a.x = d_x.p; a.fwd = d_fwd.p; a.rev_off = d_off.p; a.rev = d_rev.p; a.row_ids = d_rows.p; a.err = err ? d_err.p : nullptr;
        a.rows = 1; a.D = (uint32_t)D; a.R = R; a.alpha = alpha; a.tau = tau; a.alpha_max = alpha_max;
        a.out = d_out.p; a.out_cnt = d_cnt.p;
        hipLaunchKernelGGL(build::select_kernel, dim3(1), dim3(64), build::select_lds(a.D), nullptr, a);
        HIP_CHECK(hipGetLastError());
        HIP_CHECK(hipDeviceSynchronize());
        HIP_CHECK(hipMemcpy(out_ids, d_out.p, 128, hipMemcpyDeviceToHost));
        HIP_CHECK(hipMemcpy(out_cnt, d_cnt.p, 4, hipMemcpyDeviceToHost));
    });
}

int cph_calib_hook(cph_index* h, const float* queries, const uint32_t* start, uint64_t ns, float* rec, uint32_t* rec_cnt,
                   float* dqp) {
    return guarded([&] {
        if (!h || !queries || !start || !rec || !rec_cnt || !dqp || ns == 0 || ns > 0xFFFFFFull) throw InvalidArg("bad arguments");
        std::lock_guard<std::mutex> lk(h->mu);
        require_finalized(h);
        for (uint64_t i = 0; i < ns; ++i)
            if (start[i] >= h->host.n) throw InvalidArg("start vertex out of range");
        h->use_device();
        hipStream_t st = own_stream(h);
        BatchSet& s = next_set(h, st);
        stage_queries(h, s, upload_queries(h, s, queries, ns, st), ns, st);
        HIP_CHECK(hipEventRecord(s.ev_done, st));
        s.used = true;
        DevBuf<uint32_t> d_start(ns), d_rc(ns);
        DevBuf<float> d_rec(ns * 32 * 6), d_dqp(ns);
        HIP_CHECK(hipMemcpyAsync(d_start.p, start, ns * 4, hipMemcpyHostToDevice, st));
        build::CalibArgs c{};
        c.blocks = h->d_blocks.p; c.raw = h->d_raw.p; c.L = h->L; c.n = h->host.n;
        c.queries = s.d_queries.p; c.qmasks = s.d_qmasks.p; c.qhdr = s.d_qhdr.p;
        c.start = d_start.p; c.ns = (uint32_t)ns; c.rec = d_rec.p; c.rec_cnt = d_rc.p; c.dqp_out = d_dqp.p;
        const size_t lds = (size_t)h->L.PW * 16 + (size_t)h->L.D * 8;
        const dim3 grid((uint32_t)std::min<uint64_t>(ns, (uint64_t)h->num_cus * 16));
        if (h->bits == 1) hipLaunchKernelGGL(build::calib_kernel<1>, grid, dim3(64), lds, st, c);
        else if (h->bits == 2) hipLaunchKernelGGL(build::calib_kernel<2>, grid, dim3(64), lds, st, c);
        else hipLaunchKernelGGL(build::calib_kernel<4>, grid, dim3(64), lds, st, c);
        HIP_CHECK(hipGetLastError());
        HIP_CHECK(hipEventRecord(s.ev_done, st));
        HIP_CHECK(hipStreamSynchronize(st));
        HIP_CHECK(hipMemcpy(rec, d_rec.p, ns * 32 * 6 * 4, hipMemcpyDeviceToHost));
        HIP_CHECK(hipMemcpy(rec_cnt, d_rc.p, ns * 4, hipMemcpyDeviceToHost));
        HIP_CHECK(hipMemcpy(dqp, d_dqp.p, ns * 4, hipMemcpyDeviceToHost));
    });
}

int cph_get_vectors(cph_index* h, uint64_t first, uint64_t count, float* out) {
    return guarded([&] {
        if (!h || !out) throw InvalidArg("null argument");
        refuse_host_less(h, "cph_get_vectors");
        std::lock_guard<std::mutex> lk(h->mu);
        require_finalized(h);
        if (first + count > h->host.n) throw InvalidArg("vector range out of bounds");
        for (uint64_t i = 0; i < count; ++i)
            std::memcpy(out + i * h->dim, h->host.vec(first + i), h->dim * sizeof(float));
    });
}

int cph_set_search_params(cph_index* h, uint32_t slots, uint64_t beam_capacity) {
    return guarded([&] {
        std::lock_guard<std::mutex> lk(h->mu);
        h->want_slots = slots;
        h->want_cap = beam_capacity;
    });
}

int cph_set_batch_sets(cph_index* h, uint32_t n_sets) {
    return guarded([&] {
        if (!h) throw InvalidArg("null handle");
        if (n_sets < 1 || n_sets > (uint32_t)kMaxBatchSets) throw InvalidArg("n_sets must be 1.." + std::to_string(kMaxBatchSets));
        std::lock_guard<std::mutex> lk(h->mu);
        h->use_device();
        quiesce(h);
        for (int i = (int)n_sets; i < kMaxBatchSets; ++i) release_scratch(h->sets[i]);
        h->n_sets = (int)n_sets;
        h->last_set = (int)n_sets - 1;
    });
}

int cph_last_search_stats(cph_index* h, uint64_t out[12]) {
    return guarded([&] {
        if (!h || !out) throw InvalidArg("null argument");
        std::lock_guard<std::mutex> lk(h->mu);
        for (int i = 0; i < 12; ++i) out[i] = 0;
        if (h->last_range) {
            out[kStatExact] = h->range_exact;
            return;
        }
        if (h->last_search < 0) return;
        BatchSet& s = h->sets[h->last_search];
        h->use_device();
        HIP_CHECK(hipEventSynchronize(s.ev_done));
        if (s.stats_in_hbm) {
            HIP_CHECK(hipMemcpy(s.pin_stats, s.d_stats.p, kStatWords * 8, hipMemcpyDeviceToHost));
            s.stats_in_hbm = false;
        }
        float ms = 0.0f;
        HIP_CHECK(hipEventElapsedTime(&ms, s.ev0, s.ev1));
        for (int i = kStatExpansions; i <= kStatAllSeen; ++i) out[i] = s.pin_stats[i];
        out[kStatNoCounter] = (uint64_t)(ms * 1000.0);
        out[8] = s.run_slots;
        out[9] = s.run_cap;
        out[10] = stage2_stat(s, kStatStage2Reruns);
        out[11] = stage2_stat(s, kStatStage2Undecided);
#if defined(CPH_PHASE_TIMERS) || defined(CPH_TRAFFIC_STATS)
        const unsigned long long* diag = s.pin_stats + kStatDiag;
#endif
#if CPH_PHASE_TIMERS + 0 == 2
        fprintf(stderr, "[fine cycles] head+issue=%llu pop=%llu block_wait=%llu probe_issue+exact+nnpush=%llu estimator=%llu probe_wait=%llu mark+cand=%llu pushes+tail=%llu\n",
                diag[0], diag[1], diag[2], diag[3], diag[4], diag[5], diag[6], diag[7]);
#elif defined(CPH_PHASE_TIMERS)
        fprintf(stderr, "[phase cycles] pop=%llu load+exact+nnpush=%llu sums+epi=%llu atomic+log+stage=%llu spec_exact=%llu replay=%llu tail=%llu other=%llu\n",
                diag[0], diag[1], diag[2], diag[3], diag[4], diag[5], diag[6], diag[7]);
#endif
#ifdef CPH_TRAFFIC_STATS
        fprintf(stderr, "[traffic] hybrid_pops=%llu windows=%llu hybrid_pushes=%llu hbm_appends=%llu probe_lines=%llu sum_beam_at_pop=%llu max_beam=%llu pops_beyond_8191=%llu\n",
                diag[0], diag[1], diag[2], diag[3], diag[4], diag[5], diag[6], diag[7]);
#endif
    });
}

int cph_last_query_expansions(cph_index* h, uint32_t* out, uint64_t n) {
    return guarded([&] {
        if (!h || !out) throw InvalidArg("null argument");
        std::lock_guard<std::mutex> lk(h->mu);
        if (h->last_search < 0 || n != h->sets[h->last_search].nq)
            throw InvalidArg("n must equal the size of the last batch");
        BatchSet& s = h->sets[h->last_search];
        h->use_device();
        HIP_CHECK(hipEventSynchronize(s.ev_done));
        HIP_CHECK(hipMemcpy(out, s.d_status.p, n * sizeof(uint32_t), hipMemcpyDeviceToHost));
        for (uint64_t i = 0; i < n; ++i) out[i] >>= 8;
    });
}

int cph_synchronize(cph_index* h) {
    return guarded([&] {
        if (!h) throw InvalidArg("null handle");
        std::lock_guard<std::mutex> lk(h->mu);
        h->use_device();
        quiesce(h);
    });
}

int cph_order_queries(cph_index* h, const float* keys, uint64_t n, uint32_t* order) {
    return guarded([&] {
        if (!h || !keys || !order) throw InvalidArg("null argument");
        if (n == 0 || n > 0xFFFFFFFFull) throw InvalidArg("bad n");
        std::lock_guard<std::mutex> lk(h->mu);
        h->use_device();
        DevBuf<float> dk;
        DevBuf<uint32_t> dord;
        dk.alloc(n);
        dord.alloc(n);
        HIP_CHECK(hipMemcpy(dk.p, keys, n * 4, hipMemcpyHostToDevice));
        hipLaunchKernelGGL(order_kernel, dim3(1), dim3(1024), 0, nullptr, dk.p, (uint32_t)n, dord.p);
        HIP_CHECK(hipGetLastError());
        HIP_CHECK(hipMemcpy(order, dord.p, n * 4, hipMemcpyDeviceToHost));
    });
}

int cph_search_batch(cph_index* h, const float* queries, uint64_t n, uint64_t k, int64_t* ids,
                     float* dist) {
    return guarded([&] { search_batch_host(h, queries, n, k, nullptr, ids, dist); });
}

int cph_search_batch_device(cph_index* h, const float* d_queries, uint64_t n, uint64_t k,
                            int64_t* d_ids, float* d_dist, void* stream) {
    return guarded([&] { search_batch_device(h, d_queries, n, k, nullptr, d_ids, d_dist, stream); });
}

int cph_filter_create(cph_index* h, const uint32_t* words, uint64_t n_bits, cph_filter** out) {
    return guarded([&] {
        if (!h || !out || (!words && n_bits != 0)) throw InvalidArg("null argument");
        *out = nullptr;
        if (n_bits > 0xFFFFFFFFull) throw InvalidArg("filter too large");
        const uint64_t nw = (n_bits + 31) / 32;
        std::vector<uint32_t> w(words, words + nw);
        if (n_bits & 31) w[nw - 1] &= (1u << (n_bits & 31)) - 1u;
        uint64_t pc = 0;
        for (uint32_t x : w) pc += (uint64_t)__builtin_popcount(x);
        std::unique_ptr<cph_filter> f(new cph_filter());
        f->device = h->device;
        f->n_bits = n_bits;
        f->popcount = pc;
        h->use_device();
        f->words.alloc(std::max<uint64_t>(nw, 1));
        if (nw) HIP_CHECK(hipMemcpy(f->words.p, w.data(), nw * 4, hipMemcpyHostToDevice));
        *out = f.release();
    });
}

int cph_filter_destroy(cph_filter* f) {
    return guarded([&] {
        if (!f) return;
        std::unique_ptr<cph_filter> own(f);
        HIP_CHECK(hipSetDevice(f->device));
        HIP_CHECK(hipDeviceSynchronize());
    });
}

int cph_search_batch_filtered(cph_index* h, const float* queries, uint64_t n, uint64_t k, const cph_filter* f,
                              int64_t* ids, float* dist) {
    return guarded([&] { search_batch_host(h, queries, n, k, f, ids, dist); });
}

int cph_search_batch_device_filtered(cph_index* h, const float* d_queries, uint64_t n, uint64_t k, const cph_filter* f,
                                     int64_t* d_ids, float* d_dist, void* stream) {
    return guarded([&] { search_batch_device(h, d_queries, n, k, f, d_ids, d_dist, stream); });
}

int cph_search_batch_exact(cph_index* h, const float* queries, uint64_t n, uint64_t k, const cph_filter* f, int64_t* ids,
                           float* dist) {
    return guarded([&] { search_batch_host(h, queries, n, k, f, ids, dist, true); });
}

int cph_search_batch_exact_device(cph_index* h, const float* d_queries, uint64_t n, uint64_t k, const cph_filter* f,
                                  int64_t* d_ids, float* d_dist, void* stream) {
    return guarded([&] { search_batch_device(h, d_queries, n, k, f, d_ids, d_dist, stream, true); });
}

int cph_search_batch_filters(cph_index* h, const float* queries, uint64_t n, uint64_t k, const cph_filter* const* filters,
                             uint32_t n_filters, const int32_t* filter_of, int exact, int64_t* ids, float* dist) {
    return guarded([&] { search_batch_filters_host(h, queries, n, k, filters, n_filters, filter_of, exact != 0, ids, dist); });
}

int cph_search_batch_filters_device(cph_index* h, const float* d_queries, uint64_t n, uint64_t k, const cph_filter* const* filters,
                                    uint32_t n_filters, const int32_t* filter_of, int exact, int64_t* d_ids, float* d_dist,
                                    void* stream) {
    return guarded([&] {
        search_batch_filters_device(h, d_queries, n, k, filters, n_filters, filter_of, exact != 0, d_ids, d_dist, stream);
    });
}

int cph_host_filter_groups(const int32_t* filter_of, uint64_t n, const uint64_t* popcounts, uint32_t n_filters, uint64_t k, int exact,
                           uint64_t exact_threshold, uint8_t* routes, uint32_t* perm, uint32_t* seg) {
    return guarded([&] {
        if (!routes || !seg || (n && (!filter_of || !perm)) || (n_filters && !popcounts)) throw InvalidArg("null argument");
        if (n > 0xFFFFFFFFull) throw InvalidArg("batch too large");
        filter_groups(filter_of, n, popcounts, n_filters, k, exact != 0, exact_threshold, routes, perm, seg);
    });
}

int cph_host_exact_group_plan(const uint64_t* seg_candidates, const uint64_t* seg_queries, uint32_t n_segments, uint64_t k, int num_cus,
                              uint64_t scratch_bytes, uint32_t* items, uint64_t cap_items, uint64_t* out) {
    return guarded([&] {
        if (!out || (n_segments && (!seg_candidates || !seg_queries)) || (cap_items && !items)) throw InvalidArg("null argument");
        if (k == 0 || k > kExactMaxK) throw InvalidArg("exact plan: sizes out of range");
        for (uint32_t s = 0; s < n_segments; ++s)
            if (seg_candidates[s] > 0xFFFFFFFFull || seg_queries[s] > 0xFFFFFFFFull) throw InvalidArg("exact plan: sizes out of range");
        const ExactGroupPlan pl = plan_exact_groups(seg_candidates, seg_queries, n_segments, (uint32_t)k, num_cus, (size_t)scratch_bytes);
        out[0] = pl.items.size(); out[1] = pl.launch_pools.size(); out[2] = pl.gq; out[3] = pl.C;
        out[4] = (uint64_t)pl.max_pools * pl.C * 8; out[5] = 0;
        for (size_t i = 0; i < pl.items.size() && i < cap_items; ++i) {
            const ExactGroupItem& it = pl.items[i];
            const uint32_t row[8] = {it.seg, it.part, it.c_lo, it.c_hi, it.q_lo, it.q_cnt, it.pool, it.launch};
            std::memcpy(items + i * 8, row, sizeof(row));
        }
    });
}

int cph_set_exact_threshold(cph_index* h, uint64_t max_allowed) {
    return guarded([&] {
        if (!h) throw InvalidArg("null handle");
        std::lock_guard<std::mutex> lk(h->mu);
        h->exact_threshold = max_allowed;
    });
}

int cph_host_filter_ids(const uint32_t* words, uint64_t n_bits, uint32_t* out_ids, uint64_t* out_count) {
    return guarded([&] {
// ... 2286 lines not shown
```

rabitq-ann-search_amd/csrc/device_search.h:

```cpp
#pragma once
#include <cstddef>
#include <hip/hip_runtime.h>

#include "cph_core.h"
#include "device_fastscan.h"

namespace cph {

struct Result {
    uint32_t id;
    float dist;
};

enum StatWord : int {
    kStatExpansions = 0,
    kStatExact = 1,
    kStatNew = 2,
    kStatPushes = 3,
    kStatSkips = 4,
    kStatReruns = 5,
    kStatNoCounter = 6,
    kStatAllSeen = 7,
    kStatStage2Reruns = 8,
    kStatStage2Undecided = 9,
    kStatDiag = 8,
#if defined(CPH_PHASE_TIMERS) || defined(CPH_TRAFFIC_STATS)
    kStatFlushed = 8,
#else
    kStatFlushed = 10,
#endif
    kStatQueues = 16,
    kStatWords = 20,
};
enum StatQueueWord : int {
    kQueueMain = 0,
    kQueueRerunLen = 1,
    kQueueRerun = 2,
    kQueueSecond = 3,
};

struct SearchArgs {
    const uint8_t* blocks;
    const float* raw;
    const float* norm_sq;
    uint64_t n;
    DevLayout L;
    uint32_t flags;
    const float* queries;
    const uint4* qmasks;
    const QueryHeader* qhdr;
    const uint32_t* todo;
    uint32_t nq;
    const uint32_t* nq_dev;
    uint32_t k;
    SearchConsts sc;
    uint32_t* counter;
    uint64_t cap;
    uint64_t bm_words;
    uint32_t* bitmaps;
    uint32_t* beam_pages;
    uint32_t* beam_tail;
    uint32_t* log_ids;
    int64_t* out_ids;
    float* out_dist;
    uint32_t* out_count;
    uint32_t* status;
    unsigned long long* stats;
    uint32_t* redo;
    uint32_t* redo_count;
    uint32_t* done_flags;
    uint32_t done_seq;
    const uint32_t* allow;
    const uint32_t* rows;
    const uint32_t* const* allow_tab;
    const uint32_t* filter_of;
};

template <class T>
__device__ __forceinline__ T cold_arg(size_t offset) {
    typedef __attribute__((address_space(4))) const unsigned char kbyte;
    kbyte* p = (kbyte*)__builtin_amdgcn_kernarg_segment_ptr();
    asm volatile("" : "+s"(p));
    return *(__attribute__((address_space(4))) const T*)(p + offset);
}
#define CPH_COLD(field) cold_arg<decltype(SearchArgs::field)>(offsetof(SearchArgs, field))

__device__ __forceinline__ void nn_sift_up(Result* h, uint32_t hole, uint32_t top, Result v) {
    while (hole > top) {
        uint32_t p = (hole - 1) >> 1;
        Result pv = h[p];
        if (!(pv.dist < v.dist)) break;
        h[hole] = pv;
        hole = p;
    }
    h[hole] = v;
}
__device__ __forceinline__ void nn_adjust(Result* h, uint32_t hole, uint32_t len, Result v) {
    const uint32_t top = hole;
    uint32_t child = hole;
    while (child < (len - 1) / 2) {
        child = 2 * (child + 1);
        Result r = h[child], l = h[child - 1];
        if (r.dist < l.dist) { --child; r = l; }
        h[hole] = r;
        hole = child;
    }
    if ((len & 1) == 0 && child == (len - 2) / 2) {
        child = 2 * (child + 1);
        h[hole] = h[child - 1];
        hole = child - 1;
    }
    nn_sift_up(h, hole, top, v);
}
__device__ __forceinline__ void nn_push(Result* h, uint32_t& size, uint32_t k, Result r) {
    if (size < k) {
        nn_sift_up(h, size, 0, r);
        ++size;
    } else if (r.dist < h[0].dist) {
        if (size > 1) {
            Result v = h[size - 1];
            nn_adjust(h, 0, size - 1, v);
        }
        nn_sift_up(h, size - 1, 0, r);
    }
}
__device__ __forceinline__ void nn_sort(Result* h, uint32_t size) {
    while (size > 1) {
        Result v = h[size - 1];
        h[size - 1] = h[0];
        nn_adjust(h, 0, size - 1, v);
        --size;
    }
}

constexpr uint32_t kBeamLds = 255;
constexpr uint32_t kBeamPaged = 8191;
constexpr uint32_t kPageDwords = 192;
constexpr uint32_t kBeamPagesDwords = 128 * kPageDwords;
__host__ __device__ inline size_t beam_tail_dwords(uint64_t cap) {
    const size_t d = 3 * (size_t)(cap > kBeamPaged ? cap - kBeamPaged : 0) + 4;
    return (d + 31) & ~(size_t)31;
}

struct BeamEntry {
    float est, lower;
    uint32_t id;
};

__device__ __forceinline__ int opaque_lane(int lane) {
    asm volatile("" : "+v"(lane));
    return lane;
}

typedef uint32_t u32x4 __attribute__((ext_vector_type(4)));
typedef uint32_t u32x3 __attribute__((ext_vector_type(3)));
typedef __attribute__((address_space(3))) u32x4 lds_u32x4;
typedef __attribute__((address_space(3))) float lds_f32;
typedef __attribute__((address_space(3))) uint32_t lds_u32;

__device__ __forceinline__ uint32_t beam_page_off(uint32_t i) {
    const uint32_t hp = i + 1;
    const uint32_t l = ((31u - (uint32_t)__builtin_clz(hp)) - 7u) & 7u;
    const uint32_t r = (hp & ((1u << l) - 1u)) | (1u << l);
    return ((hp >> l) - 128u) * kPageDwords + 3u * r;
}
__device__ __forceinline__ uint32_t beam_tail_off(uint32_t i) { return 3u * (i - kBeamPaged); }

struct Beam {
    typedef uint4 E;
    lds_u32x4* l;
    uint32_t* gp;
    uint32_t* gt;
    static __device__ __forceinline__ bool before(float a, float b) { return a > b; }
    static __device__ __forceinline__ float key_of(uint4 e) { return __uint_as_float(e.x); }
    __device__ __forceinline__ uint4 lds(uint32_t i) const {
        const u32x4 t = l[i];
        return make_uint4(t.x, t.y, t.z, t.w);
// ... 130 lines not shown
__device__ __forceinline__ void heap_push_wave(const H& h, uint32_t hole, typename H::E v, int lane_in) {
#ifdef CPH_LAUNDER_HOT
    const int lane = opaque_lane(lane_in);
#else
    const int lane = lane_in;
#endif
    const uint32_t hp = hole + 1;
    const uint32_t depth = 31u - (uint32_t)__builtin_clz(hp);
    const uint32_t t = (uint32_t)lane + 1;
    const bool on = t <= depth;
    const uint32_t pt = on ? (hp >> t) - 1 : 0u;
    const typename H::E e = h.lds(pt);
    const bool down = on && H::before(H::key_of(e), H::key_of(v));
    const unsigned long long stop = ~__ballot(down);
    const uint32_t m = (uint32_t)__builtin_ctzll(stop);
    if (t <= m) h.lds_put((hp >> (t - 1)) - 1, e);
    if ((uint32_t)lane == m) h.lds_put((hp >> m) - 1, v);
}

__device__ __forceinline__ void beam_pop_hybrid(const Beam& h, uint32_t size, int lane_in) {
    const int lane = opaque_lane(lane_in);
    const uint32_t len = size - 1;
    const uint4 v = Beam::load3(h.spill_ptr(len));
    const bool b0 = Beam::before(h.lds_key(2 * lane + 2), h.lds_key(2 * lane + 1));
    const unsigned long long m0 = __ballot(b0);
    bool b1 = false;
    if (lane < 63) b1 = Beam::before(h.lds_key(2 * lane + 130), h.lds_key(2 * lane + 129));
    const unsigned long long m1 = __ballot(b1);
    uint32_t hp = 1, d = 7;
    {
        const unsigned long long ms0 = m0 << 1, ms1 = (m1 << 1) | (m0 >> 63);
        asm volatile(
            "s_bitcmp0_b64 %[a], %[hp]\n\ts_addc_u32 %[hp], %[hp], %[hp]\n\t"
            "s_bitcmp0_b64 %[a], %[hp]\n\ts_addc_u32 %[hp], %[hp], %[hp]\n\t"
            "s_bitcmp0_b64 %[a], %[hp]\n\ts_addc_u32 %[hp], %[hp], %[hp]\n\t"
            "s_bitcmp0_b64 %[a], %[hp]\n\ts_addc_u32 %[hp], %[hp], %[hp]\n\t"
            "s_bitcmp0_b64 %[a], %[hp]\n\ts_addc_u32 %[hp], %[hp], %[hp]\n\t"
            "s_bitcmp0_b64 %[a], %[hp]\n\ts_addc_u32 %[hp], %[hp], %[hp]\n\t"
            "s_bitcmp0_b64 %[b], %[hp]\n\ts_addc_u32 %[hp], %[hp], %[hp]"
            : [hp] "+s"(hp)
            : [a] "s"(ms0), [b] "s"(ms1)
            : "scc");
    }
    const uint32_t r = (uint32_t)lane + 2;
    const uint32_t dr = 31u - (uint32_t)__builtin_clz(r);
    auto walk = [&](float key, uint32_t idx) {
        const float key_r = __shfl_down(key, 1);
        const bool both = (lane & 1) == 0 && lane < 62 && idx + 1 < len;
        const unsigned long long E2 = __ballot(both) << 2;
        const unsigned long long M = __ballot(both && Beam::before(key_r, key)) << 2;
        uint32_t P = 1, tmp;
        asm volatile(
            "1:\n\t"
            "s_lshl_b32 %[t], %[P], 1\n\t"
            "s_bitcmp1_b64 %[e], %[t]\n\t"
            "s_cbranch_scc0 2f\n\t"
            "s_bitcmp0_b64 %[m], %[t]\n\t"
            "s_addc_u32 %[P], %[P], %[P]\n\t"
            "s_cmp_lt_u32 %[P], 32\n\t"
            "s_cbranch_scc1 1b\n\t"
            "2:"
            : [P] "+s"(P), [t] "=&s"(tmp)
            : [e] "s"(E2), [m] "s"(M)
            : "scc");
        const uint32_t steps = 31u - (uint32_t)__builtin_clz(P);
        hp = (hp << steps) | (P & ((1u << steps) - 1u));
        d += steps;
        return steps;
    };
    const uint32_t pbase = (hp - 128u) * kPageDwords;
    uint4 w = make_uint4(0u, 0u, 0u, 0u);
    uint32_t steps = 0;
    if (2 * hp - 1 < len) {
        const uint32_t idx = ((hp << dr) | (r & ((1u << dr) - 1u))) - 1u;
        if (lane < 62 && idx < len) w = h.pload(pbase + 3u * r);
        steps = walk(__uint_as_float(w.x), idx);
    }
    while (steps == 5 && 2 * hp < len) {
        const uint32_t idx = ((hp << dr) | (r & ((1u << dr) - 1u))) - 1u;
        float key = 0.0f;
        if (lane < 62 && idx < len) key = __uint_as_float(h.gt[beam_tail_off(idx)]);
        steps = walk(key, idx);
    }
    if (2 * hp == len) {
        hp = 2 * hp;
        ++d;
    }
    const uint32_t t = (uint32_t)lane < d ? (uint32_t)lane : 0u;
    const uint32_t dst_hp = hp >> (d - t);
    const uint32_t src_hp = hp >> (d - t - ((uint32_t)lane < d ? 1u : 0u));
    auto page_rel = [](uint32_t node_hp, uint32_t lvl) {
        return (node_hp & ((1u << lvl) - 1u)) | (1u << lvl);
    };
    auto put_level = [&](uint32_t level, uint32_t node_hp, uint4 val) {
        if (level <= 7) h.lds_put(node_hp - 1, val);
        else if (level <= 12) h.pstore(pbase + 3u * page_rel(node_hp, level - 7u), val);
        else h.tstore(beam_tail_off(node_hp - 1), val);
    };
    const bool from_page = (uint32_t)lane < d && t >= 7 && t <= 11;
    const int page_lane = (int)page_rel(src_hp, from_page ? t - 6u : 1u) - 2;
    const uint4 pw = make_uint4((uint32_t)__shfl((int)w.x, page_lane), (uint32_t)__shfl((int)w.y, page_lane),
                                (uint32_t)__shfl((int)w.z, page_lane), 0u);
    uint4 e = v;
    bool c = false;
    if ((uint32_t)lane < d) {
        if (t < 7) e = h.lds(src_hp - 1);
        else if (t <= 11) e = pw;
        else e = h.tload(beam_tail_off(src_hp - 1));
        c = Beam::before(Beam::key_of(e), Beam::key_of(v));
    }
    const unsigned long long stay = ~__ballot(c) & ((1ull << d) - 1ull);
    const uint32_t fin = stay ? 64u - (uint32_t)__builtin_clzll(stay) : 0u;
    if ((uint32_t)lane < fin) put_level(t, dst_hp, e);
    if (fin == d) { if (lane == 0) put_level(d, hp, v); }
    else if ((uint32_t)lane == fin) put_level(t, dst_hp, v);
}

__device__ __forceinline__ void beam_push_hybrid(const Beam& h, uint32_t hole, uint4 v, int lane_in) {
    const int lane = opaque_lane(lane_in);
    const uint32_t hp = hole + 1;
    const uint32_t depth = 31u - (uint32_t)__builtin_clz(hp);
    const uint32_t t = (uint32_t)lane + 1;
    const bool on = t <= depth;
    uint4 e = v;
    bool down = false;
    if (hp <= kBeamPaged) {
        const uint32_t lvl = depth - 7u;
        const uint32_t pbase = ((hp >> lvl) - 128u) * kPageDwords;
        const uint32_t rl = (hp & ((1u << lvl) - 1u)) | (1u << lvl);
        if (on) {
            if (t < lvl) e = h.pload(pbase + 3u * (rl >> t)); else e = h.lds((hp >> t) - 1);
            down = Beam::before(Beam::key_of(e), Beam::key_of(v));
        }
        const unsigned long long stop = ~__ballot(down);
        const uint32_t m = (uint32_t)__builtin_ctzll(stop);
        auto put_anc = [&](uint32_t s, uint4 val) {
            if (s < lvl) h.pstore(pbase + 3u * (rl >> s), val); else h.lds_put((hp >> s) - 1, val);
        };
        if (t <= m) put_anc(t - 1, e);
        if ((uint32_t)lane == m) put_anc(m, v);
        return;
    }
    const uint32_t pt = on ? (hp >> t) - 1 : 0u;
    if (on) {
        e = h.raw(pt);
        down = Beam::before(Beam::key_of(e), Beam::key_of(v));
    }
    const unsigned long long stop = ~__ballot(down);
    const uint32_t m = (uint32_t)__builtin_ctzll(stop);
    if (t <= m) h.put((hp >> (t - 1)) - 1, e);
    if ((uint32_t)lane == m) h.put((hp >> m) - 1, v);
}

__device__ __forceinline__ void nn_push_wave(const NnLds& w, Result* h, uint32_t& size, uint32_t k, uint32_t id, float dist,
                                             float top, int lane_in) {
#ifndef CPH_NO_LAUNDER_NN
    const int lane = opaque_lane(lane_in);
#else
    const int lane = lane_in;
#endif
    const uint2 r = make_uint2(id, __float_as_uint(dist));
    if (size < k) {
        if (size < kWaveHeapMax) {
            heap_push_wave(w, size, r, lane);
        } else {
            if (lane == 0) nn_sift_up(h, size, 0, Result{id, dist});
            __builtin_amdgcn_wave_barrier();
        }
        ++size;
    } else if (dist < top) {
        if (size <= kWaveHeapMax) {
            if (size > 1) heap_pop_wave(w, size, lane);
            heap_push_wave(w, size - 1, r, lane);
        } else {
            if (lane == 0) {
                nn_adjust(h, 0, size - 1, h[size - 1]);
                nn_sift_up(h, size - 1, 0, Result{id, dist});
            }
            __builtin_amdgcn_wave_barrier();
        }
    }
}

__device__ __forceinline__ uint32_t bcast_u32(uint32_t v) {
    return (uint32_t)__builtin_amdgcn_readfirstlane((int)v);
}
__device__ __forceinline__ float bcast_f32(float v) {
    return __uint_as_float((uint32_t)__builtin_amdgcn_readfirstlane((int)__float_as_uint(v)));
}

constexpr uint32_t kLdsTail = 128 + 64 + 128 + 16 + 80;
__host__ __device__ inline uint32_t search_vec_bytes(uint32_t D, bool static_d) { return static_d ? D * 4 : 512; }
__host__ __device__ inline bool search_static_d(uint32_t D) { return D == 128 || D == 1024; }
__host__ __device__ inline size_t search_lds_bytes(uint32_t D, uint32_t PW, uint32_t k) {
    return (size_t)PW * 16 + (size_t)D * 4 + search_vec_bytes(D, search_static_d(D)) + kLdsTail +
           (((size_t)k * 8 + 15) & ~(size_t)15) + 16 * (kBeamLds + 1);
}

typedef __attribute__((address_space(3))) void lds_void;
__device__ __forceinline__ uint32_t lds_offset(const void* p) {
    return (uint32_t)__builtin_amdgcn_readfirstlane((int)(uint32_t)(uintptr_t)(lds_void*)p);
}
__device__ __forceinline__ void lds_dma16(const void* g, uint32_t lds_off) {
    asm volatile("s_mov_b32 m0, %1\n\ts_nop 0\n\tglobal_load_lds_dwordx4 %0, off" ::"v"(g), "s"(lds_off) : "memory");
}

#ifndef CPH_SEARCH_WAVES_PER_SIMD
#define CPH_SEARCH_WAVES_PER_SIMD 5
#endif
#ifndef CPH_SEARCH_WAVES_PER_SIMD_128
#define CPH_SEARCH_WAVES_PER_SIMD_128 6
#endif
#ifndef CPH_SEARCH_WAVES_PER_SIMD_1024
#define CPH_SEARCH_WAVES_PER_SIMD_1024 2
#endif
#ifndef CPH_SEARCH_WAVES_PER_SIMD_128_NARROW
#define CPH_SEARCH_WAVES_PER_SIMD_128_NARROW CPH_SEARCH_WAVES_PER_SIMD_128
#endif
__host__ __device__ constexpr int search_waves_per_simd(int sd, int bw) {
    return sd == 128 ? (bw <= 2 ? CPH_SEARCH_WAVES_PER_SIMD_128_NARROW : CPH_SEARCH_WAVES_PER_SIMD_128)
                     : (sd == 1024 ? CPH_SEARCH_WAVES_PER_SIMD_1024 : CPH_SEARCH_WAVES_PER_SIMD);
}
template <int BW, int SD, bool PF = true, bool FILT = false, bool FTAB = false>
__global__ __launch_bounds__(64, search_waves_per_simd(SD, BW)) void search_kernel(SearchArgs a) {
    extern __shared__ __align__(16) unsigned char smem[];
    const int lane = threadIdx.x;
    const int li = lane & 31;
    const uint32_t D = SD ? SD : a.L.D;
    const uint32_t PW = SD ? (SD >= 32 ? SD / 32 : 1) : a.L.PW;
    const uint32_t k = a.k;
    uint4* qm = reinterpret_cast<uint4*>(smem);
    float* qv = reinterpret_cast<float*>(smem + (size_t)PW * 16);
    unsigned char* fixed = smem + (size_t)PW * 16 + (size_t)D * 4;
    float* s_vec = reinterpret_cast<float*>(fixed);
    constexpr uint32_t vsz = SD >= 128 ? (uint32_t)SD * 4u : 512u;
    float* s_exact = reinterpret_cast<float*>(fixed + vsz);
    uint8_t* s_list = fixed + vsz + 128;
    float* s_slack = reinterpret_cast<float*>(fixed + vsz + 192);
    double* s_ratio = reinterpret_cast<double*>(fixed + vsz + 320);
    unsigned long long* s_tot = reinterpret_cast<unsigned long long*>(fixed + vsz + 336);
    if (lane < 10) s_tot[lane] = 0ull;
    Result* nn = reinterpret_cast<Result*>(fixed + vsz + kLdsTail);
    NnLds nnw;
    nnw.l = (lds_u32x2*)(fixed + vsz + kLdsTail);
    const uint32_t beam_off = PW * 16 + D * 4 + vsz + kLdsTail + ((k * 8 + 15) & ~15u);
    lds_u32x4* s_beam = (lds_u32x4*)(smem + beam_off);

    const uint32_t vec_off = __builtin_amdgcn_groupstaticsize() + PW * 16 + D * 4;
    const uint32_t slot = blockIdx.x;
    uint32_t* bm = CPH_COLD(bitmaps) + (size_t)slot * CPH_COLD(bm_words);
    uint32_t* logi = CPH_COLD(log_ids) + (size_t)slot * a.cap;
    Beam heap;
    heap.l = s_beam;
    heap.gp = CPH_COLD(beam_pages) + (size_t)slot * kBeamPagesDwords;
    heap.gt = CPH_COLD(beam_tail) + (size_t)slot * beam_tail_dwords(a.cap);
    const float FMAX = 3.402823466e+38f;
    if (lane < kMaxSlack) s_slack[lane] = a.sc.slack[lane];

    const uint32_t* nq_dev = CPH_COLD(nq_dev);
    const uint32_t nq = nq_dev ? *nq_dev : CPH_COLD(nq);
    for (;;) {
        uint32_t t = 0;
        if (lane == 0) t = atomicAdd(CPH_COLD(counter), 1u);
        t = bcast_u32(t);
        if (t >= nq) break;
        const uint32_t* todo = CPH_COLD(todo);
        const uint32_t qi = todo ? todo[t] : t;

        {
            const uint4* qmasks = CPH_COLD(qmasks);
            const float* queries = CPH_COLD(queries);
            for (uint32_t w = lane; w < PW; w += 64) qm[w] = qm_lds_word(qmasks[(size_t)qi * PW + w], nib_codes<BW, SD>(a.L));
            for (uint32_t d = lane; d < D; d += 64) qv[d] = queries[(size_t)qi * D + d];
        }
        const QueryHeader hd = CPH_COLD(qhdr)[qi];
        const uint32_t* allow_q = nullptr;
        if constexpr (FTAB) allow_q = CPH_COLD(allow_tab)[CPH_COLD(filter_of)[qi]];
        __syncthreads();

        QP qp;
        qp.A = hd.A; qp.B = hd.B; qp.C = hd.C;
        {
            float af_a = a.sc.affine_a, af_b = a.sc.affine_b, fl = a.sc.ip_qo_floor;
            asm volatile("" : "+s"(af_a), "+s"(af_b), "+s"(fl));
            qp.affine_a = af_a; qp.affine_b = af_b; qp.floor = fl;
        }
        qp.slack = s_slack[0];
        const float gamma = a.sc.gamma;

        float qnorm;
        {
            float c = 0.0f;
            for (uint32_t i = lane & 7; i < D; i += 8) c = __fmaf_rn(qv[i], qv[i], c);
            qnorm = bcast_f32(group_reduce8_lo(c));
        }

        uint32_t beam_size = 0, nn_size = 0;
        float gamma_q = gamma;
        if (lane == 0) { s_ratio[0] = 0.0; s_ratio[1] = 0.0; nn[0].dist = FMAX; }
        uint32_t ratio_count = 0;
        uint32_t log_count = 0;
        int slack_batch = 0;
        bool overflow = false, wipe = false, stage2_redo = false;
        uint32_t st_exp = 0, st_exact = 0, st_new = 0, st_push = 0, st_skip = 0, st_allseen = 0;
        uint32_t st_undecided = 0;
#ifdef CPH_TRAFFIC_STATS
        unsigned long long trf[8] = {0, 0, 0, 0, 0, 0, 0, 0};
#endif
#ifdef CPH_PHASE_TIMERS
        unsigned long long tph[8] = {0, 0, 0, 0, 0, 0, 0, 0};
        unsigned long long tlast = clock64();
#define CPH_TICK_(i) do { unsigned long long tn_ = clock64(); tph[i] += tn_ - tlast; tlast = tn_; } while (0)
#if CPH_PHASE_TIMERS + 0 == 2
#define CPH_TICK(i) do {} while (0)
#define CPH_TICKF(i) CPH_TICK_(i)
#else
#define CPH_TICK(i) CPH_TICK_(i)
#define CPH_TICKF(i) do {} while (0)
#endif
#else
#define CPH_TICK(i) do {} while (0)
#define CPH_TICKF(i) do {} while (0)
#endif

        {
            const uint32_t ep = hd.entry;
            const float enorm = a.norm_sq[ep];
            float dot = group_dot8_lo(qv, a.raw + (size_t)ep * D, D, lane & 7);
            float ex = exact_from_dot(qnorm, enorm, dot);
            st_exact++;
            if (lane == 0) {
                logi[0] = ep;
                heap.put(0, beam_pack(BeamEntry{ex, 0.0f, ep}));
                atomicOr(&bm[ep >> 5], 1u << (ep & 31));
            }
            beam_size = 1;
            log_count = 1;
        }
        __syncthreads();

        for (;;) {
            CPH_TICK(7);
            if (beam_size == 0) break;
            uint32_t cur_id;
            float worst_pop;
            auto pop_beam = [&](uint32_t size) {
#ifdef CPH_TRAFFIC_STATS
                trf[5] += size;
                if (size > trf[6]) trf[6] = size;
                if (size > kBeamLds) { trf[0]++; uint32_t lv = 31u - (uint32_t)__builtin_clz(size); trf[1] += (lv - 7 + 4) / 5; }
                if (size > 8191) trf[7]++;
#endif
                if (size > 1) {
                    if (size <= kBeamLds) heap_pop_wave(heap, size, lane);
                    else beam_pop_hybrid(heap, size, lane);
                }
            };
            {
                const uint4 topv = heap.lds(0);
                const float worst = nn[0].dist;
                cur_id = bcast_u32(topv.z);
                const float cur_est = __uint_as_float(topv.x);
                const float cur_lower = __uint_as_float(topv.y);
                uint32_t verdict = 2;
                if (nn_size >= k && cur_est >= gamma_q * worst) verdict = 0;
                else if (nn_size >= k && cur_lower > worst) verdict = 1;
                verdict = bcast_u32(verdict);
                if (verdict == 0) break;
                if (verdict == 1) {
                    pop_beam(beam_size);
                    --beam_size;
                    continue;
                }
                worst_pop = bcast_f32(worst);
            }
            CPH_TICK(0);

            constexpr bool kStaticLayout = SD >= 128 && PF;
            const uint32_t blk_stride = kStaticLayout ? StaticLayout<BW, SD>::kStride : a.L.stride;
            const uint32_t blk_ids_off = kStaticLayout ? StaticLayout<BW, SD>::kIdsOff : a.L.ids_off;
            const uint8_t* blk = a.blocks + (size_t)cur_id * blk_stride;
            const float* vrow = a.raw + (size_t)cur_id * D;
#ifndef CPH_NO_LOOPHEAD_WAIT
            __builtin_amdgcn_s_waitcnt(0x0F70);
#endif
            if constexpr (SD == 128) {
                if (lane < 32) lds_dma16(vrow + 4 * lane, vec_off);
                __builtin_amdgcn_sched_barrier(0);
            } else if constexpr (SD > 128) {
#pragma unroll
                for (int c = 0; c < SD / 256; ++c) lds_dma16(vrow + 4 * lane + 256 * c, vec_off + 1024 * c);
                __builtin_amdgcn_sched_barrier(0);
            }
            const float norm_ld = a.norm_sq[cur_id];
            const uint32_t nid_ld = reinterpret_cast<const uint32_t*>(blk + blk_ids_off)[li];
            uint32_t allow_cur = 0;
            if constexpr (FTAB) allow_cur = allow_q[cur_id >> 5];
            else if constexpr (FILT) allow_cur = CPH_COLD(allow)[cur_id >> 5];
            BlockLoads<BW, SD> bl;
#ifdef CPH_NO_PROBE_FIRST
            constexpr bool kProbeFirst = false;
#else
            constexpr bool kProbeFirst = PF && SD >= 128;
#endif
            if constexpr (kProbeFirst) {
#pragma unroll
                for (int kk = 0; kk < BlockLoads<BW, SD>::kCPL; ++kk) bl.c[kk] = make_uint4(0u, 0u, 0u, 0u);
                bl.aux = make_uint4(0u, 0u, 0u, 0u);
            } else {
                bl.issue(blk, a.L, lane);
            }
            __builtin_amdgcn_sched_barrier(0);
            CPH_TICKF(0);
            uint32_t touch = 0;
            if (beam_size > kBeamLds) {
                const uint32_t depth = 31u - (uint32_t)__builtin_clz(beam_size);
                const uint32_t j = (uint32_t)lane + 1u;
                const bool on = j <= 5u && 7u + j < depth;
                const uint32_t sh = on ? depth - 7u - j : 0u;
                const uint32_t rj = ((beam_size >> sh) & ((1u << (j & 7u)) - 1u)) | (1u << (j & 7u));
                const uint32_t pb = ((beam_size >> (depth - 7u)) - 128u) * kPageDwords;
                touch = heap.gp[on ? pb + 3u * rj : 0u];
            }
            pop_beam(beam_size);
            --beam_size;
            __builtin_amdgcn_sched_barrier(0);
            CPH_TICKF(1);
            uint32_t nid = nid_ld;
            float cur_norm = norm_ld;
            float dot_generic = 0.0f;
            if constexpr (SD < 128) dot_generic = bcast_f32(group_dot8_lo(qv, vrow, D, lane & 7));
            if constexpr (!kProbeFirst) bl.retire();
            asm volatile("" : "+v"(cur_norm), "+v"(nid) : "v"(touch));
            CPH_TICKF(2);
            const bool valid = nid != kInvalidNode;
            const bool active = lane < 32 && valid;
            uint32_t old_bits = 0;
            const uint32_t my_bit = 1u << (nid & 31);
            old_bits = __hip_atomic_load(&bm[active ? nid >> 5 : 0u], __ATOMIC_RELAXED, __HIP_MEMORY_SCOPE_AGENT);
            __builtin_amdgcn_sched_barrier(0);
#ifdef CPH_TRAFFIC_STATS
            {
                const uint32_t line = nid >> 10;
                bool first = active;
                for (int j = 0; j < 31; ++j) {
                    const uint32_t oj = __shfl(line, j);
                    const bool aj = __shfl((int)active, j) != 0;
                    if (aj && lane > j && oj == line) first = false;
                }
                trf[4] += __popcll(__ballot(first));
            }
#endif

            float exact_dist;
            {
                float dot;
                if constexpr (SD >= 128) dot = bcast_f32(group_reduce8_lo(chain_dot_lds<SD / 8>(qv, s_vec, lane & 7, 0.0f)));
                else dot = dot_generic;
                exact_dist = exact_from_dot(qnorm, cur_norm, dot);
            }
            st_exact++;
            st_exp++;
            float worst0 = worst_pop;
            const bool cur_allowed = !FILT || ((allow_cur >> (cur_id & 31u)) & 1u) != 0u;
            const bool nn_changes = bcast_u32((cur_allowed && (nn_size < k || exact_dist < worst_pop)) ? 1u : 0u) != 0u;
            if (nn_changes) {
                nn_push_wave(nnw, nn, nn_size, k, cur_id, exact_dist, worst_pop, lane);
                __builtin_amdgcn_wave_barrier();
                worst0 = bcast_f32(nnw.lds_key(0));
            }
            const uint32_t nn_sz = nn_size;
            CPH_TICK(1);
            CPH_TICKF(3);
            if (!__any(active)) {
                asm volatile("" ::"v"(old_bits));
                continue;
            }

            if (a.sc.num_slack > 0) {
                int lvl = slack_batch < a.sc.num_slack - 1 ? slack_batch : a.sc.num_slack - 1;
                qp.slack = s_slack[lvl];
                ++slack_batch;
            }
            float est = 0.0f, lower = 0.0f;
            bool skipped2 = false, undecided2 = false;
            const TailLanes tl = kProbeFirst ? no_tail() : tail_lanes(valid, lane);
            auto estimate = [&](bool fetched) -> bool {
                LaneEst v;
                const float dqp = exact_dist;
                const float sq = __builtin_sqrtf(dqp);
                bl.reduce(blk, a.L, qm, lane, v);
                if constexpr (BW == 1) {
                    stage2_est<1>(qp, v, dqp, sq, est, lower, tl);
                } else {
                    float lo1 = 0.0f, lo2 = 0.0f;
                    const bool tiny = bcast_f32(dqp) < kEpsSmall;
                    if (!tiny) lower_bounds_split<BW>(qp, v, dqp, sq, lane, lo1, lo2, tl);
                    if (__builtin_expect(nn_sz < k || __any(fetched && valid && lo1 < worst0), 1)) {
                        est = stage2_est_only<BW>(qp, v, dqp, tl, tiny);
                        lower = lo2;
                    } else if constexpr (!kProbeFirst) {
                        est = FMAX;
                        lower = lo1;
                        skipped2 = true;
                    } else {
                        LaneEst w = v;
                        asm volatile("" : "+v"(w.nbit));
                        est = stage2_est_only<BW>(qp, w, dqp, tl, tiny);
                        lower = lo2;
                        const bool acts = fetched && !(lo2 >= worst0) && (est < worst0 || est < gamma_q * worst0);
                        if (__any(acts)) return false;
                        undecided2 = true;
                    }
                }
                return true;
            };
            constexpr bool kSpeculate = BW <= 2 && !kProbeFirst;
            if constexpr (kSpeculate) estimate(true);
            CPH_TICKF(4);
#if CPH_PHASE_TIMERS + 0 == 2
            asm volatile("" : "+v"(old_bits));
            CPH_TICKF(5);
#endif

            bool is_new = active && (old_bits & my_bit) == 0;
            if ((a.flags & 1u) && __any(is_new)) {
#pragma unroll 1
                for (int j = 0; j < 31; ++j) {
                    uint32_t oj = __shfl(nid, j);
                    bool nj = __shfl((int)is_new, j) != 0;
                    if (nj && lane > j && lane < 32 && oj == nid) is_new = false;
                }
            }
            const uint32_t new_mask = (uint32_t)(__ballot(is_new) & 0xFFFFFFFFull);
            const uint32_t n_new = __popc(new_mask);
            const uint32_t my_rank = __builtin_amdgcn_mbcnt_lo(new_mask, 0u);
            if (beam_size + n_new > a.cap) { overflow = true; break; }
            if (!wipe && log_count + n_new > a.cap) wipe = true;
            if (is_new) {
                atomicOr(&bm[nid >> 5], my_bit);
                if (!wipe) logi[log_count + my_rank] = nid;
            }
            if (new_mask == 0) {
                ++st_allseen;
                continue;
            }
            if constexpr (kProbeFirst) {
                const bool fetch = ((new_mask >> (lane & 31)) & 1u) != 0u;
                if (fetch) bl.issue_static(blk, lane);
                if (__builtin_expect(!estimate(fetch), 0)) { overflow = true; stage2_redo = true; break; }
            } else if constexpr (!kSpeculate) {
                estimate(true);
            }
            if (skipped2) st_skip++;
            if (undecided2) st_undecided++;

            CPH_TICK(2);
            const bool warmup = nn_sz < k;
            bool cand = is_new && (warmup || (!(lower >= worst0) && est < worst0));
            const uint32_t cand_mask = (uint32_t)(__ballot(cand) & 0xFFFFFFFFull);

            st_new += n_new;
            CPH_TICK(3);

            uint32_t allow_mask = 0;
            if (cand_mask) {
                uint32_t allow_w = 0;
                if constexpr (FTAB) allow_w = allow_q[is_new ? nid >> 5 : 0u];
                else if constexpr (FILT) allow_w = CPH_COLD(allow)[is_new ? nid >> 5 : 0u];
                if (cand) s_list[__builtin_amdgcn_mbcnt_lo(cand_mask, 0u)] = (uint8_t)lane;
                __syncthreads();
                const uint32_t n_cand = __popc(cand_mask);
                const int g = lane >> 3;
                for (uint32_t base = 0; base < n_cand; base += 8) {
                    const bool have = base + g < n_cand;
                    const uint32_t idx = have ? s_list[base + g] : 0;
                    const uint32_t cid_l = (uint32_t)__shfl((int)nid, (int)idx);
                    const uint32_t cid = have ? cid_l : cur_id;
                    const float cnorm = a.norm_sq[cid];
                    float dot = group_dot8_lo(qv, a.raw + (size_t)cid * D, D, lane & 7);
                    float ex = exact_from_dot(qnorm, cnorm, dot);
                    asm volatile("" ::"v"(ex));
                    if (have && (lane & 7) == 0) s_exact[idx] = ex;
                }
                st_exact += n_cand;
                __syncthreads();
                if constexpr (FILT) allow_mask = (uint32_t)(__ballot(is_new && ((allow_w >> (nid & 31u)) & 1u) != 0u) & 0xFFFFFFFFull);
            }
            CPH_TICK(4);
            CPH_TICKF(6);

            if (!warmup && cand_mask == 0) {
                const float dabs0 = gamma_q * worst0;
                const bool p = is_new && !(lower >= worst0) && est < dabs0;
                uint32_t pm = (uint32_t)(__ballot(p) & 0xFFFFFFFFull);
                const uint32_t np = __popc(pm);
                bool appended = false;
#ifdef CPH_NO_SKIP_APPEND
                if (np != 0 && np <= beam_size + 1) {
#else
                if (np != 0 && np <= beam_size + 1 && !(np == 1 && beam_size >= kBeamLds)) {
#endif
                    const uint32_t pos = beam_size + __builtin_amdgcn_mbcnt_lo(pm, 0u);
                    const bool in_lds = beam_size + np <= kBeamLds;
                    bool stay = true;
                    if (in_lds) {
                        const bool chk = p && pos > 0;
                        stay = !(heap.lds_key(chk ? (pos - 1) >> 1 : 0u) > est) || !chk;
                    } else if (p && pos > 0) {
                        stay = !(heap.raw_key((pos - 1) >> 1) > est);
                    }
                    if (__all(stay)) {
#ifdef CPH_TRAFFIC_STATS
                        if (!in_lds) trf[3]++;
#endif
                        const uint4 ent = make_uint4(__float_as_uint(est), __float_as_uint(lower), nid, 0u);
                        if (p) { if (in_lds) heap.lds_put(pos, ent); else heap.put(pos, ent); }
                        beam_size += np;
                        st_push += np;
                        appended = true;
                    }
                }
                if (!appended) {
                    while (pm) {
                        const int i = __ffs((int)pm) - 1;
                        pm &= pm - 1;
                        const uint32_t id_i = (uint32_t)__builtin_amdgcn_readlane((int)nid, i);
                        const uint32_t e_i = (uint32_t)__builtin_amdgcn_readlane((int)__float_as_uint(est), i);
                        const uint32_t lo_i = (uint32_t)__builtin_amdgcn_readlane((int)__float_as_uint(lower), i);
#ifdef CPH_TRAFFIC_STATS
                        if (beam_size >= kBeamLds) trf[2]++;
#endif
                        if (beam_size < kBeamLds) heap_push_wave(heap, beam_size, make_uint4(e_i, lo_i, id_i, 0u), lane);
                        else beam_push_hybrid(heap, beam_size, make_uint4(e_i, lo_i, id_i, 0u), lane);
                        ++beam_size;
                        ++st_push;
                    }
                }
            } else {
                uint32_t m = warmup ? new_mask
                                    : new_mask & (uint32_t)(__ballot(!(lower >= worst0)) & 0xFFFFFFFFull);
                while (m) {
                    const int i = __ffs((int)m) - 1;
                    m &= m - 1;
                    const uint32_t id_i = (uint32_t)__builtin_amdgcn_readlane((int)nid, i);
                    const float e = __uint_as_float((uint32_t)__builtin_amdgcn_readlane((int)__float_as_uint(est), i));
                    const float lo_i = __uint_as_float((uint32_t)__builtin_amdgcn_readlane((int)__float_as_uint(lower), i));
                    const float worst = bcast_f32(nnw.lds_key(0));
                    const float dabs = (nn_size >= k) ? gamma_q * worst : FMAX;
                    uint32_t act = 0;
                    if (warmup) act = 1;
                    else if (!(lo_i >= worst)) act = (e < worst) ? 5u : ((e < dabs) ? 2u : 0u);
                    act = bcast_u32(act);
                    float key = e, lo = lo_i;
                    bool push = (act & 2u) != 0;
                    if (act & 1u) {
                        const float ex = bcast_f32(s_exact[i]);
                        if (!FILT || ((allow_mask >> i) & 1u) != 0u) nn_push_wave(nnw, nn, nn_size, k, id_i, ex, worst, lane);
                        if (ex < dabs) { push = true; key = ex; if (warmup) lo = ex; }
                        if ((act & 4u) && ex > kEpsSmall) {
                            ++ratio_count;
                            if (lane == 0) {
                                double r = (double)(e / ex);
                                const double rs = s_ratio[0] + r;
                                const double rq = fma(r, r, s_ratio[1]);
                                s_ratio[0] = rs;
                                s_ratio[1] = rq;
                                if (ratio_count >= a.sc.gamma_warmup) {
                                    double cnt = (double)ratio_count;
                                    double mean = rs / cnt;
                                    double var = fma(-mean, mean, rq / cnt);
                                    double sd = sqrt(var < 0.0 ? 0.0 : var);
                                    float gq = gamma * (float)fma((double)a.sc.gamma_beta, sd, 1.0);
                                    gamma_q = (gq < gamma) ? gamma
                                                           : ((a.sc.gamma_max < gq) ? a.sc.gamma_max : gq);
                                }
                            }
                            gamma_q = bcast_f32(gamma_q);
                        }
                    }
                    if (bcast_u32(push ? 1u : 0u)) {
                        const uint4 ent = beam_pack(BeamEntry{key, lo, id_i});
#ifdef CPH_TRAFFIC_STATS
                        if (beam_size >= kBeamLds) trf[2]++;
#endif
                        if (beam_size < kBeamLds) heap_push_wave(heap, beam_size, ent, lane);
                        else beam_push_hybrid(heap, beam_size, ent, lane);
                        ++beam_size;
                        ++st_push;
                    }
                }
                CPH_TICK(4);
            }
            CPH_TICK(5);
            log_count += n_new;
            __builtin_amdgcn_wave_barrier();
            CPH_TICK(6);
            CPH_TICKF(7);
        }

        if (lane == 0 && !overflow) nn_sort(nn, nn_size);
        const uint32_t nn_final = bcast_u32(nn_size);
        __syncthreads();
        if (!overflow) {
            int64_t* out_ids = CPH_COLD(out_ids);
            float* out_dist = CPH_COLD(out_dist);
            const uint32_t* rows = CPH_COLD(rows);
            for (uint32_t j = lane; j < k; j += 64) {
                if (j < nn_final) {
                    out_ids[(size_t)qi * k + j] = (int64_t)(rows ? rows[nn[j].id] : nn[j].id);
                    out_dist[(size_t)qi * k + j] = nn[j].dist;
                } else {
                    out_ids[(size_t)qi * k + j] = -1;
                    out_dist[(size_t)qi * k + j] = FMAX;
                }
            }
        }
        if (lane == 0) {
            CPH_COLD(out_count)[qi] = nn_final;
            CPH_COLD(status)[qi] = (overflow ? kStatusOverflow : kStatusOk) | (st_exp << 8);
            s_tot[kStatExpansions] += st_exp;
            s_tot[kStatExact] += st_exact;
            s_tot[kStatNew] += st_new;
            s_tot[kStatPushes] += st_push;
            s_tot[kStatSkips] += st_skip;
            s_tot[kStatAllSeen] += st_allseen;
            if (stage2_redo) s_tot[kStatStage2Reruns] += 1;
            s_tot[kStatStage2Undecided] += st_undecided;
#if defined(CPH_PHASE_TIMERS) || defined(CPH_TRAFFIC_STATS)
            unsigned long long* stats = CPH_COLD(stats);
#endif
#ifdef CPH_PHASE_TIMERS
            for (int i = 0; i < 8; ++i) atomicAdd(&stats[kStatDiag + i], tph[i]);
#endif
#ifdef CPH_TRAFFIC_STATS
            for (int i = 0; i < 8; ++i) { if (i == 6) atomicMax(&stats[kStatDiag + i], trf[i]); else atomicAdd(&stats[kStatDiag + i], trf[i]); }
#endif
            if (overflow) {
                s_tot[kStatReruns] += 1;
                uint32_t* redo = CPH_COLD(redo);
                if (redo) redo[atomicAdd(CPH_COLD(redo_count), 1u)] = qi;
            }
        }
        if (uint32_t* done_flags = CPH_COLD(done_flags); done_flags != nullptr && !overflow) {
            __threadfence_system();
            if (lane == 0) __hip_atomic_store(&done_flags[qi], CPH_COLD(done_seq), __ATOMIC_RELEASE, __HIP_MEMORY_SCOPE_SYSTEM);
        }
        __syncthreads();
        if (overflow || wipe) {
            const uint64_t bm_words = CPH_COLD(bm_words);
            for (uint64_t w = lane; w < bm_words; w += 64) bm[w] = 0u;
        } else {
            for (uint32_t j = lane; j < log_count; j += 64) bm[logi[j] >> 5] = 0u;
        }
        __syncthreads();
    }
    if (lane < kStatFlushed) {
        const unsigned long long v = s_tot[lane];
        if (v != 0ull && lane != kStatNoCounter) atomicAdd(&CPH_COLD(stats)[lane], v);
    }
}

}
```

Baseline: 6.149 million queries/s.

## Add lean LDS-only beam search kernel variant with adaptive fallback

Adds a LEAN template specialization of the search kernel that keeps the beam entirely in LDS, drops the HBM-spilled hybrid beam paths, the dedup loop and the wave-heap size checks. Queries whose beam would exceed LDS capacity are flagged as overflow and rerun through the normal path. A host-side adaptation disables lean mode when too many queries rerun, and base pointers are pinned to scalar registers with empty asm constraints. The cost is an occasional synchronous wait on the first lean batch and extra reruns for queries with large beams.

Result: slower. 3.465 million queries/s (-43.7%).

```diff
diff --git a/include/cphnsw_mi355x.h b/include/cphnsw_mi355x.h
--- a/include/cphnsw_mi355x.h
+++ b/include/cphnsw_mi355x.h
@@ -111,6 +111,7 @@
 int cph_set_search_params(cph_index* h, uint32_t slots, uint64_t beam_capacity);
 
 int cph_last_search_stats(cph_index* h, uint64_t out[12]);
+int cph_last_lean_stats(cph_index* h, uint64_t out[2]);
 int cph_last_query_expansions(cph_index* index, uint32_t* out, uint64_t n);
 int cph_order_queries(cph_index* index, const float* keys, uint64_t n, uint32_t* order);
 
diff --git a/rabitq-ann-search_amd/cphnsw_mi355x/_lib.py b/rabitq-ann-search_amd/cphnsw_mi355x/_lib.py
--- a/rabitq-ann-search_amd/cphnsw_mi355x/_lib.py
+++ b/rabitq-ann-search_amd/cphnsw_mi355x/_lib.py
@@ -96,6 +96,7 @@
     "cph_get_vectors": (C.c_int, [C.c_void_p, C.c_uint64, C.c_uint64, C.c_void_p]),
     "cph_set_search_params": (C.c_int, [C.c_void_p, C.c_uint32, C.c_uint64]),
     "cph_last_search_stats": (C.c_int, [C.c_void_p, C.POINTER(C.c_uint64)]),
+    "cph_last_lean_stats": (C.c_int, [C.c_void_p, C.POINTER(C.c_uint64)]),
     "cph_last_query_expansions": (C.c_int, [C.c_void_p, C.c_void_p, C.c_uint64]),
     "cph_order_queries": (C.c_int, [C.c_void_p, C.c_void_p, C.c_uint64, C.c_void_p]),
     "cph_multi_create": (C.c_int, [C.c_uint64, C.c_uint64, C.c_void_p, C.c_uint32, C.POINTER(C.c_void_p)]),
diff --git a/rabitq-ann-search_amd/cphnsw_mi355x/index.py b/rabitq-ann-search_amd/cphnsw_mi355x/index.py
--- a/rabitq-ann-search_amd/cphnsw_mi355x/index.py
+++ b/rabitq-ann-search_amd/cphnsw_mi355x/index.py
@@ -786,7 +786,13 @@
         keys = ("expansions", "exact_l2", "new_neighbours", "beam_pushes", "stage2_skipped",
                 "rerun_queries", "kernel_us", "expansions_nothing_new", "slots", "capacity",
                 "stage2_reruns", "stage2_undecided") + (("merge_us",) if self._p is not None else ())
-        return dict(zip(keys, [int(x) for x in out]))
+        st = dict(zip(keys, [int(x) for x in out]))
+        fn = getattr(_lib.lib(), "cph_last_lean_stats", None)
+        if self._p is None and self._m is None and fn is not None:
+            lean = (C.c_uint64 * 2)()
+            _lib.check(fn(self._h, lean))
+            st["lean_main"], st["lean_handovers"] = int(lean[0]), int(lean[1])
+        return st
 
     def synchronize(self):
         for h in self._replicas():
diff --git a/rabitq-ann-search_amd/csrc/cphnsw_mi355x.hip b/rabitq-ann-search_amd/csrc/cphnsw_mi355x.hip
--- a/rabitq-ann-search_amd/csrc/cphnsw_mi355x.hip
+++ b/rabitq-ann-search_amd/csrc/cphnsw_mi355x.hip
@@ -118,6 +118,7 @@
     uint32_t nq = 0;
     uint32_t run_slots = 0;
     uint64_t run_cap = 0;
+    bool lean = false;
     DevBuf<float> x_qpad, x_qnorm;
     DevBuf<unsigned long long> x_pools;
     DevBuf<uint32_t> x_counts;
@@ -216,6 +217,9 @@
     uint64_t auto_cap = 0;
     bool pf_off = false;
     bool pf_dense = false;
+    int lean_mode = -1;
+    bool lean_off = false;
+    bool lean_proven = false;
     std::mutex mu;
     SearchCoalescer coal;
     struct LeaderSlot {
@@ -245,10 +249,17 @@
 #endif
 }
 
+bool lean_main(const cph_index* h, uint32_t k, uint64_t cap) {
+    if (h->lean_mode == 0 || (h->lean_mode != 1 && h->lean_off)) return false;
+    return probe_first(h) && !(h->flags & 1u) && k <= kWaveHeapMax && cap >= kBeamLds;
+}
+
 void reset_adaptation(cph_index* h) {
     h->auto_cap = 0;
     h->pf_off = false;
     h->pf_dense = false;
+    h->lean_off = false;
+    h->lean_proven = false;
     h->last_search = -1;
     h->last_range = false;
 }
@@ -472,11 +483,18 @@
     BatchSet& s = h->sets[h->last_set];
     init_set(s);
     for (BatchSet& o : h->sets) {
-        if (!(o.used && o.ev_done && !o.stats_in_hbm && hipEventQuery(o.ev_done) == hipSuccess)) continue;
+        if (!(o.used && o.ev_done && !o.stats_in_hbm)) continue;
+        if (o.lean && h->lean_mode == -1 && !h->lean_off && !h->lean_proven) HIP_CHECK(hipEventSynchronize(o.ev_done));
+        if (hipEventQuery(o.ev_done) != hipSuccess) continue;
         const uint64_t reruns = o.pin_stats[kStatReruns], stage2_reruns = stage2_stat(o, kStatStage2Reruns);
-        if (reruns > stage2_reruns && o.cap < h->host.n + 1)
+        const uint64_t lean_reruns = stage2_stat(o, kStatLeanReruns);
+        if (reruns > stage2_reruns + lean_reruns && o.cap < h->host.n + 1)
             h->auto_cap = std::max<uint64_t>(h->auto_cap, std::min<uint64_t>(h->host.n + 1, o.cap * 4));
         if (stage2_reruns * 50 > o.nq) h->pf_off = true;
+        if (o.lean) {
+            if (lean_reruns * 50 > o.nq) h->lean_off = true;
+            else h->lean_proven = true;
+        }
         if (o.pin_stats[kStatExpansions] >= 10000) {
             const double new_per_exp = (double)o.pin_stats[kStatNew] / (double)o.pin_stats[kStatExpansions];
             const double off = h->bits == 4 ? 6.0 : 2.8, on = h->bits == 4 ? 4.5 : 2.2;
@@ -485,6 +503,7 @@
         }
     }
     if (s.used) HIP_CHECK(hipStreamWaitEvent(st, s.ev_done, 0));
+    s.lean = false;
     return s;
 }
 
@@ -572,9 +591,14 @@
     Direct,
 };
 
-void launch_search_kernel(uint32_t bits, uint32_t D, bool pf, bool filtered, bool table_of_filters, uint32_t grid, size_t lds,
-                          hipStream_t st, const SearchArgs& a) {
+void launch_search_kernel(uint32_t bits, uint32_t D, bool pf, bool filtered, bool table_of_filters, bool lean, uint32_t grid,
+                          size_t lds, hipStream_t st, const SearchArgs& a) {
     using Kernel = void (*)(SearchArgs);
+    static const Kernel lean_table[3][2] = {
+        {search_kernel<1, 128, true, false, false, true>, search_kernel<1, 1024, true, false, false, true>},
+        {search_kernel<2, 128, true, false, false, true>, search_kernel<2, 1024, true, false, false, true>},
+        {search_kernel<4, 128, true, false, false, true>, search_kernel<4, 1024, true, false, false, true>},
+    };
     static const Kernel table[3][3][4] = {
         {{search_kernel<1, 0, true, false>, search_kernel<1, 0, true, false>, search_kernel<1, 0, false, true>,
           search_kernel<1, 0, false, true, true>},
@@ -595,7 +619,11 @@
          {search_kernel<4, 1024, false, false>, search_kernel<4, 1024, true, false>, search_kernel<4, 1024, false, true>,
           search_kernel<4, 1024, false, true, true>}},
     };
-    const Kernel kernel = table[bits == 1 ? 0 : bits == 2 ? 1 : 2][D == 128 ? 1 : D == 1024 ? 2 : 0][table_of_filters ? 3 : filtered ? 2 : pf ? 1 : 0];
+    Kernel kernel = table[bits == 1 ? 0 : bits == 2 ? 1 : 2][D == 128 ? 1 : D == 1024 ? 2 : 0][table_of_filters ? 3 : filtered ? 2 : pf ? 1 : 0];
+    if (lean) {
+        if (!pf || filtered || table_of_filters || !(D == 128 || D == 1024)) throw std::logic_error("lean search launch without its conditions");
+        kernel = lean_table[bits == 1 ? 0 : bits == 2 ? 1 : 2][D == 128 ? 0 : 1];
+    }
     hipLaunchKernelGGL(kernel, dim3(grid), dim3(64), lds, st, a);
     HIP_CHECK(hipGetLastError());
 }
@@ -614,6 +642,8 @@
     const uint64_t n = h->host.n;
     const bool tab = sub && sub->allow_tab;
     const bool pf = mode == Launch::Main && d_allow == nullptr && !tab && probe_first(h);
+    const bool lean = pf && sub == nullptr && done.flags == nullptr && lean_main(h, k, s.cap);
+    if (mode != Launch::Rerun) s.lean = lean;
     SearchArgs a{};
     a.allow = d_allow;
     if (tab) { a.allow_tab = sub->allow_tab; a.filter_of = sub->filter_of; }
@@ -677,7 +707,7 @@
     }
     const size_t lds = search_lds_bytes(h->L.D, h->L.PW, k);
     if (lds > 160 * 1024) throw InvalidArg("k too large for the on-chip result heap");
-    launch_search_kernel(h->bits, h->L.D, pf, d_allow != nullptr, tab, grid, lds, st, a);
+    launch_search_kernel(h->bits, h->L.D, pf, d_allow != nullptr, tab, lean, grid, lds, st, a);
 }
 
 void finish_batch(cph_index* h, BatchSet& s, hipStream_t st) {
@@ -738,6 +768,7 @@
     }
     s.d_stats.alloc(kStatWords);
     HIP_CHECK(hipMemsetAsync(s.d_stats.p, 0, kStatWords * 8, st));
+    s.lean = false;
     if (filter && filter->popcount == 0) {
         uint32_t* d_count = d_count_out ? d_count_out : s.d_count.p;
         HIP_CHECK(hipEventRecord(s.ev0, st));
@@ -1294,6 +1325,7 @@
         if (const char* e = getenv("CPH_EXACT_SCRATCH_MB")) h->exact_scratch_bytes = (size_t)std::max(1, atoi(e)) << 20;
         if (const char* e = getenv("CPH_GATHER_US")) h->coal.gather_us = std::max(0, atoi(e));
         if (const char* e = getenv("CPH_WAVES_PER_CU")) { h->waves_per_cu = (uint32_t)std::max(1, atoi(e)); h->waves_from_env = true; }
+        if (const char* e = getenv("CPH_LEAN_MAIN")) h->lean_mode = e[0] == '1' ? 1 : e[0] == '0' ? 0 : -1;
         *out = h;
     });
 }
@@ -1802,6 +1834,24 @@
         fprintf(stderr, "[traffic] hybrid_pops=%llu windows=%llu hybrid_pushes=%llu hbm_appends=%llu probe_lines=%llu sum_beam_at_pop=%llu max_beam=%llu pops_beyond_8191=%llu\n",
                 diag[0], diag[1], diag[2], diag[3], diag[4], diag[5], diag[6], diag[7]);
 #endif
+    });
+}
+
+int cph_last_lean_stats(cph_index* h, uint64_t out[2]) {
+    return guarded([&] {
+        if (!h || !out) throw InvalidArg("null argument");
+        std::lock_guard<std::mutex> lk(h->mu);
+        out[0] = out[1] = 0;
+        if (h->last_range || h->last_search < 0) return;
+        BatchSet& s = h->sets[h->last_search];
+        h->use_device();
+        HIP_CHECK(hipEventSynchronize(s.ev_done));
+        if (s.stats_in_hbm) {
+            HIP_CHECK(hipMemcpy(s.pin_stats, s.d_stats.p, kStatWords * 8, hipMemcpyDeviceToHost));
+            s.stats_in_hbm = false;
+        }
+        out[0] = s.lean ? 1 : 0;
+        out[1] = stage2_stat(s, kStatLeanReruns);
     });
 }
 
diff --git a/rabitq-ann-search_amd/csrc/device_search.h b/rabitq-ann-search_amd/csrc/device_search.h
--- a/rabitq-ann-search_amd/csrc/device_search.h
+++ b/rabitq-ann-search_amd/csrc/device_search.h
@@ -23,6 +23,7 @@
     kStatAllSeen = 7,
     kStatStage2Reruns = 8,
     kStatStage2Undecided = 9,
+    kStatLeanReruns = 10,
     kStatDiag = 8,
 #if defined(CPH_PHASE_TIMERS) || defined(CPH_TRAFFIC_STATS)
     kStatFlushed = 8,
@@ -459,6 +460,7 @@
     if ((uint32_t)lane == m) h.put((hp >> m) - 1, v);
 }
 
+template <bool WAVE_ONLY = false>
 __device__ __forceinline__ void nn_push_wave(const NnLds& w, Result* h, uint32_t& size, uint32_t k, uint32_t id, float dist,
                                              float top, int lane_in) {
 #ifndef CPH_NO_LAUNDER_NN
@@ -476,7 +478,7 @@
         }
         ++size;
     } else if (dist < top) {
-        if (size <= kWaveHeapMax) {
+        if (WAVE_ONLY || size <= kWaveHeapMax) {
             if (size > 1) heap_pop_wave(w, size, lane);
             heap_push_wave(w, size - 1, r, lane);
         } else {
@@ -528,8 +530,9 @@
     return sd == 128 ? (bw <= 2 ? CPH_SEARCH_WAVES_PER_SIMD_128_NARROW : CPH_SEARCH_WAVES_PER_SIMD_128)
                      : (sd == 1024 ? CPH_SEARCH_WAVES_PER_SIMD_1024 : CPH_SEARCH_WAVES_PER_SIMD);
 }
-template <int BW, int SD, bool PF = true, bool FILT = false, bool FTAB = false>
+template <int BW, int SD, bool PF = true, bool FILT = false, bool FTAB = false, bool LEAN = false>
 __global__ __launch_bounds__(64, search_waves_per_simd(SD, BW)) void search_kernel(SearchArgs a) {
+    static_assert(!LEAN || (PF && SD >= 128 && !FILT && !FTAB), "lean: probe first, static D, unfiltered");
     extern __shared__ __align__(16) unsigned char smem[];
     const int lane = threadIdx.x;
     const int li = lane & 31;
@@ -559,8 +562,13 @@
     uint32_t* logi = CPH_COLD(log_ids) + (size_t)slot * a.cap;
     Beam heap;
     heap.l = s_beam;
-    heap.gp = CPH_COLD(beam_pages) + (size_t)slot * kBeamPagesDwords;
-    heap.gt = CPH_COLD(beam_tail) + (size_t)slot * beam_tail_dwords(a.cap);
+    if constexpr (LEAN) {
+        heap.gp = nullptr;
+        heap.gt = nullptr;
+    } else {
+        heap.gp = CPH_COLD(beam_pages) + (size_t)slot * kBeamPagesDwords;
+        heap.gt = CPH_COLD(beam_tail) + (size_t)slot * beam_tail_dwords(a.cap);
+    }
     const float FMAX = 3.402823466e+38f;
     if (lane < kMaxSlack) s_slack[lane] = a.sc.slack[lane];
 
@@ -594,6 +602,13 @@
         }
         qp.slack = s_slack[0];
         const float gamma = a.sc.gamma;
+        const uint8_t* g_blocks = a.blocks;
+        const float* g_raw = a.raw;
+        const float* g_norm = a.norm_sq;
+        uint32_t* bmq = bm;
+        asm volatile("" : "+s"(g_blocks), "+s"(g_raw), "+s"(g_norm), "+s"(bmq));
+        uint64_t cap_q = a.cap;
+        asm volatile("" : "+s"(cap_q));
 
         float qnorm;
         {
@@ -608,7 +623,7 @@
         uint32_t ratio_count = 0;
         uint32_t log_count = 0;
         int slack_batch = 0;
-        bool overflow = false, wipe = false, stage2_redo = false;
+        bool overflow = false, wipe = false, stage2_redo = false, lean_redo = false;
         uint32_t st_exp = 0, st_exact = 0, st_new = 0, st_push = 0, st_skip = 0, st_allseen = 0;
         uint32_t st_undecided = 0;
 #ifdef CPH_TRAFFIC_STATS
@@ -632,14 +647,14 @@
 
         {
             const uint32_t ep = hd.entry;
-            const float enorm = a.norm_sq[ep];
-            float dot = group_dot8_lo(qv, a.raw + (size_t)ep * D, D, lane & 7);
+            const float enorm = g_norm[ep];
+            float dot = group_dot8_lo(qv, g_raw + (size_t)ep * D, D, lane & 7);
             float ex = exact_from_dot(qnorm, enorm, dot);
             st_exact++;
             if (lane == 0) {
                 logi[0] = ep;
-                heap.put(0, beam_pack(BeamEntry{ex, 0.0f, ep}));
-                atomicOr(&bm[ep >> 5], 1u << (ep & 31));
+                heap.lds_put(0, beam_pack(BeamEntry{ex, 0.0f, ep}));
+                atomicOr(&bmq[ep >> 5], 1u << (ep & 31));
             }
             beam_size = 1;
             log_count = 1;
@@ -659,7 +674,7 @@
                 if (size > 8191) trf[7]++;
 #endif
                 if (size > 1) {
-                    if (size <= kBeamLds) heap_pop_wave(heap, size, lane);
+                    if (LEAN || size <= kBeamLds) heap_pop_wave(heap, size, lane);
                     else beam_pop_hybrid(heap, size, lane);
                 }
             };
@@ -686,8 +701,8 @@
             constexpr bool kStaticLayout = SD >= 128 && PF;
             const uint32_t blk_stride = kStaticLayout ? StaticLayout<BW, SD>::kStride : a.L.stride;
             const uint32_t blk_ids_off = kStaticLayout ? StaticLayout<BW, SD>::kIdsOff : a.L.ids_off;
-            const uint8_t* blk = a.blocks + (size_t)cur_id * blk_stride;
-            const float* vrow = a.raw + (size_t)cur_id * D;
+            const uint8_t* blk = g_blocks + (size_t)cur_id * blk_stride;
+            const float* vrow = g_raw + (size_t)cur_id * D;
 #ifndef CPH_NO_LOOPHEAD_WAIT
             __builtin_amdgcn_s_waitcnt(0x0F70);
 #endif
@@ -699,7 +714,7 @@
                 for (int c = 0; c < SD / 256; ++c) lds_dma16(vrow + 4 * lane + 256 * c, vec_off + 1024 * c);
                 __builtin_amdgcn_sched_barrier(0);
             }
-            const float norm_ld = a.norm_sq[cur_id];
+            const float norm_ld = g_norm[cur_id];
             const uint32_t nid_ld = reinterpret_cast<const uint32_t*>(blk + blk_ids_off)[li];
             uint32_t allow_cur = 0;
             if constexpr (FTAB) allow_cur = allow_q[cur_id >> 5];
@@ -720,7 +735,7 @@
             __builtin_amdgcn_sched_barrier(0);
             CPH_TICKF(0);
             uint32_t touch = 0;
-            if (beam_size > kBeamLds) {
+            if (!LEAN && beam_size > kBeamLds) {
                 const uint32_t depth = 31u - (uint32_t)__builtin_clz(beam_size);
                 const uint32_t j = (uint32_t)lane + 1u;
                 const bool on = j <= 5u && 7u + j < depth;
@@ -744,7 +759,7 @@
             const bool active = lane < 32 && valid;
             uint32_t old_bits = 0;
             const uint32_t my_bit = 1u << (nid & 31);
-            old_bits = __hip_atomic_load(&bm[active ? nid >> 5 : 0u], __ATOMIC_RELAXED, __HIP_MEMORY_SCOPE_AGENT);
+            old_bits = __hip_atomic_load(&bmq[active ? nid >> 5 : 0u], __ATOMIC_RELAXED, __HIP_MEMORY_SCOPE_AGENT);
             __builtin_amdgcn_sched_barrier(0);
 #ifdef CPH_TRAFFIC_STATS
             {
@@ -772,7 +787,7 @@
             const bool cur_allowed = !FILT || ((allow_cur >> (cur_id & 31u)) & 1u) != 0u;
             const bool nn_changes = bcast_u32((cur_allowed && (nn_size < k || exact_dist < worst_pop)) ? 1u : 0u) != 0u;
             if (nn_changes) {
-                nn_push_wave(nnw, nn, nn_size, k, cur_id, exact_dist, worst_pop, lane);
+                nn_push_wave<LEAN>(nnw, nn, nn_size, k, cur_id, exact_dist, worst_pop, lane);
                 __builtin_amdgcn_wave_barrier();
                 worst0 = bcast_f32(nnw.lds_key(0));
             }
@@ -831,7 +846,7 @@
 #endif
 
             bool is_new = active && (old_bits & my_bit) == 0;
-            if ((a.flags & 1u) && __any(is_new)) {
+            if (!LEAN && (a.flags & 1u) && __any(is_new)) {
 #pragma unroll 1
                 for (int j = 0; j < 31; ++j) {
                     uint32_t oj = __shfl(nid, j);
@@ -842,10 +857,14 @@
             const uint32_t new_mask = (uint32_t)(__ballot(is_new) & 0xFFFFFFFFull);
             const uint32_t n_new = __popc(new_mask);
             const uint32_t my_rank = __builtin_amdgcn_mbcnt_lo(new_mask, 0u);
-            if (beam_size + n_new > a.cap) { overflow = true; break; }
-            if (!wipe && log_count + n_new > a.cap) wipe = true;
+            if constexpr (LEAN) {
+                if (beam_size + n_new > kBeamLds) { overflow = true; lean_redo = true; break; }
+            } else {
+                if (beam_size + n_new > cap_q) { overflow = true; break; }
+            }
+            if (!wipe && log_count + n_new > cap_q) wipe = true;
             if (is_new) {
-                atomicOr(&bm[nid >> 5], my_bit);
+                atomicOr(&bmq[nid >> 5], my_bit);
                 if (!wipe) logi[log_count + my_rank] = nid;
             }
             if (new_mask == 0) {
@@ -884,8 +903,8 @@
                     const uint32_t idx = have ? s_list[base + g] : 0;
                     const uint32_t cid_l = (uint32_t)__shfl((int)nid, (int)idx);
                     const uint32_t cid = have ? cid_l : cur_id;
-                    const float cnorm = a.norm_sq[cid];
-                    float dot = group_dot8_lo(qv, a.raw + (size_t)cid * D, D, lane & 7);
+                    const float cnorm = g_norm[cid];
+                    float dot = group_dot8_lo(qv, g_raw + (size_t)cid * D, D, lane & 7);
                     float ex = exact_from_dot(qnorm, cnorm, dot);
                     asm volatile("" ::"v"(ex));
                     if (have && (lane & 7) == 0) s_exact[idx] = ex;
@@ -906,10 +925,10 @@
 #ifdef CPH_NO_SKIP_APPEND
                 if (np != 0 && np <= beam_size + 1) {
 #else
-                if (np != 0 && np <= beam_size + 1 && !(np == 1 && beam_size >= kBeamLds)) {
+                if (np != 0 && np <= beam_size + 1 && (LEAN || !(np == 1 && beam_size >= kBeamLds))) {
 #endif
                     const uint32_t pos = beam_size + __builtin_amdgcn_mbcnt_lo(pm, 0u);
-                    const bool in_lds = beam_size + np <= kBeamLds;
+                    const bool in_lds = LEAN || beam_size + np <= kBeamLds;
                     bool stay = true;
                     if (in_lds) {
                         const bool chk = p && pos > 0;
@@ -938,7 +957,7 @@
 #ifdef CPH_TRAFFIC_STATS
                         if (beam_size >= kBeamLds) trf[2]++;
 #endif
-                        if (beam_size < kBeamLds) heap_push_wave(heap, beam_size, make_uint4(e_i, lo_i, id_i, 0u), lane);
+                        if (LEAN || beam_size < kBeamLds) heap_push_wave(heap, beam_size, make_uint4(e_i, lo_i, id_i, 0u), lane);
                         else beam_push_hybrid(heap, beam_size, make_uint4(e_i, lo_i, id_i, 0u), lane);
                         ++beam_size;
                         ++st_push;
@@ -963,7 +982,7 @@
                     bool push = (act & 2u) != 0;
                     if (act & 1u) {
                         const float ex = bcast_f32(s_exact[i]);
-                        if (!FILT || ((allow_mask >> i) & 1u) != 0u) nn_push_wave(nnw, nn, nn_size, k, id_i, ex, worst, lane);
+                        if (!FILT || ((allow_mask >> i) & 1u) != 0u) nn_push_wave<LEAN>(nnw, nn, nn_size, k, id_i, ex, worst, lane);
                         if (ex < dabs) { push = true; key = ex; if (warmup) lo = ex; }
                         if ((act & 4u) && ex > kEpsSmall) {
                             ++ratio_count;
@@ -991,7 +1010,7 @@
 #ifdef CPH_TRAFFIC_STATS
                         if (beam_size >= kBeamLds) trf[2]++;
 #endif
-                        if (beam_size < kBeamLds) heap_push_wave(heap, beam_size, ent, lane);
+                        if (LEAN || beam_size < kBeamLds) heap_push_wave(heap, beam_size, ent, lane);
                         else beam_push_hybrid(heap, beam_size, ent, lane);
                         ++beam_size;
                         ++st_push;
@@ -1033,6 +1052,7 @@
             s_tot[kStatSkips] += st_skip;
             s_tot[kStatAllSeen] += st_allseen;
             if (stage2_redo) s_tot[kStatStage2Reruns] += 1;
+            if (LEAN && lean_redo) s_tot[kStatNoCounter] += 1;
             s_tot[kStatStage2Undecided] += st_undecided;
 #if defined(CPH_PHASE_TIMERS) || defined(CPH_TRAFFIC_STATS)
             unsigned long long* stats = CPH_COLD(stats);
@@ -1056,16 +1076,19 @@
         __syncthreads();
         if (overflow || wipe) {
             const uint64_t bm_words = CPH_COLD(bm_words);
-            for (uint64_t w = lane; w < bm_words; w += 64) bm[w] = 0u;
+            for (uint64_t w = lane; w < bm_words; w += 64) bmq[w] = 0u;
         } else {
-            for (uint32_t j = lane; j < log_count; j += 64) bm[logi[j] >> 5] = 0u;
+            for (uint32_t j = lane; j < log_count; j += 64) bmq[logi[j] >> 5] = 0u;
         }
         __syncthreads();
     }
     if (lane < kStatFlushed) {
         const unsigned long long v = s_tot[lane];
         if (v != 0ull && lane != kStatNoCounter) atomicAdd(&CPH_COLD(stats)[lane], v);
-    }
-}
-
-}
+#if !defined(CPH_PHASE_TIMERS) && !defined(CPH_TRAFFIC_STATS)
+        if (LEAN && v != 0ull && lane == kStatNoCounter) atomicAdd(&CPH_COLD(stats)[kStatLeanReruns], v);
+#endif
+    }
+}
+
+}
```
